# mitiko/weath3rb0i

Hardware: AMD Instinct MI355X
Metric: encode MiB/s, 64 KiB blocks, bit-exact vs CPU ref (higher is better)
Workload: dtype u32

## Files before the change

### weath3rb0i_amd/csrc/w3_predict.h

```cpp
#pragma once
#include "w3_device.h"
#include "../../include/w3hip.h"

namespace w3 {

#define W3_PF 8

#define W3_HALF_CU_LDS 81920u
template <int NW, size_t USED> struct HalfCuPad { static constexpr size_t words = (NW > 1 && USED < W3_HALF_CU_LDS) ? (W3_HALF_CU_LDS - USED + 3u) / 4u : (NW > 1 ? 0u : 1u); };
template <size_t WORDS> struct HalfCuPadDecl {
    static __device__ __forceinline__ void keep(uint64_t n) {
        __shared__ uint32_t pad_[WORDS];
        if (n == ~0ull) pad_[threadIdx.x % WORDS] = 1u;
    }
};
template <> struct HalfCuPadDecl<0> { static __device__ __forceinline__ void keep(uint64_t) {} };
#define W3_HALF_CU_PAD(NW, USED) HalfCuPadDecl<((NW) > 1 ? HalfCuPad<NW, (USED)>::words : 0u)>::keep(a.n);

struct PredictArgs {
    const uint8_t *in;
    uint64_t n;
    uint32_t block_size, nblocks;
    uint4 *P;
    const uint2 *keys;
    uint32_t *perm;
    uint2 *rec;
    uint4 *sink;
    const uint2 *rec_src;
    uint32_t *splits;
    uint32_t *job_counter;
    uint32_t hbits;
    uint32_t maxseg;
    uint32_t dbg_flags;
    unsigned long long *dbg;
    uint32_t fault_block;
};

#define W3_STAMP(slot)                                                                         \
    do {                                                                                       \
        if (a.dbg) {                                                                           \
            const unsigned long long t_ = __builtin_amdgcn_s_memtime();                        \
            if ((threadIdx.x & 63) == 0) atomicAdd(&a.dbg[slot], t_ - t_prev);                 \
            t_prev = t_;                                                                       \
        }                                                                                      \
    } while (0)

__device__ __forceinline__ uint64_t lane_lt_mask() { return (1ull << (threadIdx.x & 63)) - 1ull; }
__device__ __forceinline__ uint64_t lane_gt_mask() { return ~((2ull << (threadIdx.x & 63)) - 1ull); }

__device__ __forceinline__ uint32_t readlane_u32(uint32_t v, int k) { return (uint32_t)__builtin_amdgcn_readlane((int)v, k); }
__device__ __forceinline__ uint64_t readlane_u64(uint64_t v, int k) {
    uint32_t lo = readlane_u32((uint32_t)v, k), hi = readlane_u32((uint32_t)(v >> 32), k);
    return ((uint64_t)hi << 32) | lo;
}

template <int H>
__device__ __forceinline__ void match_windows(uint32_t w16, uint64_t M[8]) {
    uint64_t X[16];
#pragma unroll
    for (int b = 1; b < 16; b++) {
        if (b >= 1 && b <= 7 + H) {
            const bool mybit = (w16 >> b) & 1u;
            const uint64_t B = __ballot(mybit);
            X[b] = mybit ? B : ~B;
        }
    }
    if constexpr (H == 8) {
        uint64_t A2[15], A4[13];
#pragma unroll
        for (int b = 1; b <= 14; b++) A2[b] = X[b] & X[b + 1];
#pragma unroll
        for (int b = 1; b <= 12; b++) A4[b] = A2[b] & A2[b + 2];
#pragma unroll
        for (int j = 0; j < 8; j++) M[j] = A4[8 - j] & A4[12 - j];
    } else {
#pragma unroll
        for (int j = 0; j < 8; j++) {
            uint64_t m = ~0ull;
#pragma unroll
            for (int k = 0; k < H; k++) m &= X[8 - j + k];
            M[j] = m;
        }
    }
}

template <int H>
__device__ __forceinline__ void match_keys(uint2 k8, uint64_t M[8]) {
#pragma unroll
    for (int j = 0; j < 8; j++) {
        const uint32_t key = ((j < 4 ? k8.x : k8.y) >> (8 * (j & 3))) & 0xFFu;
        uint32_t mlo = 0xFFFFFFFFu, mhi = 0xFFFFFFFFu;
#pragma unroll
        for (int k = 0; k < H; k++) {
            const uint32_t sm = (uint32_t)__builtin_amdgcn_sbfe((int)key, k, 1);
            const uint64_t B = __ballot(sm != 0u);
            mlo &= ~((uint32_t)B ^ sm);
            mhi &= ~((uint32_t)(B >> 32) ^ sm);
        }
        M[j] = ((uint64_t)mhi << 32) | mlo;
    }
}

__device__ __forceinline__ uint32_t mbcnt64(uint64_t m) {
    return __builtin_amdgcn_mbcnt_hi((uint32_t)(m >> 32), __builtin_amdgcn_mbcnt_lo((uint32_t)m, 0u));
}

template <bool GROUPED>
__device__ __forceinline__ void rank_round(uint32_t c0, const uint32_t key[8], const uint64_t M[8], uint64_t seg, bool valid, bool rd,
                                           uint32_t *tbl, uint32_t p[8], uint32_t fin[8], uint32_t &wmask) {
    __asm__ volatile("" ::: "memory");
    const uint64_t gt = lane_gt_mask();
    const int lane = threadIdx.x & 63;
    wmask = 0u;
    uint32_t basev[8];
#pragma unroll
    for (int j = 0; j < 8; j++) basev[j] = tbl[j * 256 + key[j]];
#pragma unroll
    for (int j = 0; j < 8; j++) {
        const uint64_t Mj = M[j] & seg;
        const uint32_t bit = (c0 >> (7 - j)) & 1u;
        const uint64_t ones = __ballot(bit) & Mj;
        uint32_t base = basev[j];
        if constexpr (GROUPED) base = rd ? base : 0u;
        const uint32_t b0 = base & 0xFFFFu, b1 = base >> 16;
        const uint32_t n1l = mbcnt64(ones), n0l = mbcnt64(Mj) - n1l;
        uint32_t s0 = b0 + n0l, s1 = b1 + n1l;
        const bool last = valid && (Mj & gt) == 0ull;
        uint32_t f0 = s0 + (bit ^ 1u), f1 = s1 + bit;
        uint64_t satm = __ballot(last && (f0 >= 65535u || f1 >= 65535u));
        uint32_t f = f0 | (f1 << 16);
        while (satm) {
            const int k = __ffsll((long long)satm) - 1;
            const uint64_t Mc = readlane_u64(Mj, k);
            const uint64_t Oc = readlane_u64(ones, k);
            uint32_t st = readlane_u32(base, k);
            uint64_t it = Mc;
            while (it) {
                const int m = __ffsll((long long)it) - 1;
                it &= it - 1;
                if (lane == m) { s0 = st & 0xFFFFu; s1 = st >> 16; }
                st = counter_update_packed(st, (uint32_t)(Oc >> m) & 1u);
            }
            if (lane == k) f = st;
            satm &= satm - 1;
        }
        p[j] = counter_p(s0, s1);
        fin[j] = f;
        wmask |= last ? (1u << j) : 0u;
    }
    if constexpr (!GROUPED) {
#pragma unroll
        for (int j = 0; j < 8; j++)
            if ((wmask >> j) & 1u) tbl[j * 256 + key[j]] = fin[j];
        __asm__ volatile("" ::: "memory");
    }
}

#define W3_ATOMIC_LIM 65400u
#ifndef W3_ATOMIC_MAXSEG
#define W3_ATOMIC_MAXSEG 4u
#endif
typedef uint16_t w3_u16x2 __attribute__((ext_vector_type(2)));

__device__ __forceinline__ void atomic_round(uint32_t *tbl, uint32_t c0, const uint32_t key[8], bool on, uint32_t v[8]) {
#pragma unroll
    for (int j = 0; j < 8; j++) {
        const uint32_t inc = on ? (((c0 >> (7 - j)) & 1u) ? 0x10000u : 1u) : 0u;
        v[j] = __hip_atomic_fetch_add(&tbl[j * 256 + key[j]], inc, __ATOMIC_RELAXED, __HIP_MEMORY_SCOPE_WORKGROUP);
    }
}
__device__ __forceinline__ bool atomic_round_hot(const uint32_t v[8]) {
    w3_u16x2 m = __builtin_bit_cast(w3_u16x2, v[0]);
#pragma unroll
    for (int j = 1; j < 8; j++) m = __builtin_elementwise_max(m, __builtin_bit_cast(w3_u16x2, v[j]));
    return __ballot(max((uint32_t)m.x, (uint32_t)m.y) >= W3_ATOMIC_LIM) != 0ull;
}

__host__ __device__ __forceinline__ uint32_t lds_order_hash(uint32_t wave, uint32_t round, uint32_t lane) {
    uint32_t x = (wave * 64u + round) * 64u + lane + 0x9E3779B9u;
    x ^= x >> 16; x *= 0x7FEB352Du; x ^= x >> 15; x *= 0x846CA68Bu; x ^= x >> 16;
    return x;
}
__host__ __device__ __forceinline__ uint32_t lds_order_key(uint32_t wave, uint32_t h) {
    const uint32_t kind = wave & 3u;
    return kind == 0 ? 77u : kind == 1 ? (h & 7u) * 32u + 1u : kind == 2 ? (h & 255u) : (h & 2047u);
}
__global__ void __launch_bounds__(64) k_lds_order_selftest(uint32_t *old) {
    __shared__ uint32_t tbl[2048];
    const uint32_t lane = threadIdx.x;
    for (uint32_t i = lane; i < 2048u; i += 64u) tbl[i] = 0u;
    __builtin_amdgcn_wave_barrier();
    for (uint32_t r = 0; r < 32u; r++) {
        const uint32_t h = lds_order_hash(blockIdx.x, r, lane);
        old[(blockIdx.x * 32u + r) * 64u + lane] =
            __hip_atomic_fetch_add(&tbl[lds_order_key(blockIdx.x, h)], (h >> 20) & 1u ? 0x10000u : 1u, __ATOMIC_RELAXED, __HIP_MEMORY_SCOPE_WORKGROUP);
    }
}

__device__ __forceinline__ uint4 pack_p(const uint32_t p[8]) {
    return make_uint4(p[0] | (p[1] << 16), p[2] | (p[3] << 16), p[4] | (p[5] << 16), p[6] | (p[7] << 16));
}

__device__ __forceinline__ uint32_t mix_pair(uint32_t cur, uint32_t nw) {
    const uint32_t c_lo = cur & 0xFFFFu, c_hi = cur >> 16, n_lo = nw & 0xFFFFu, n_hi = nw >> 16;
    const uint32_t lo = opinion_dist(n_lo) > opinion_dist(c_lo) ? n_lo : c_lo;
    const uint32_t hi = opinion_dist(n_hi) > opinion_dist(c_hi) ? n_hi : c_hi;
    return lo | (hi << 16);
}
__device__ __forceinline__ uint4 mix_p(uint4 cur, uint4 nw) {
    return make_uint4(mix_pair(cur.x, nw.x), mix_pair(cur.y, nw.y), mix_pair(cur.z, nw.z), mix_pair(cur.w, nw.w));
}

#define W3_HD __host__ __device__ __forceinline__
#include "w3_verify.h"
#undef W3_HD
#include "w3_window.h"

template <int H, bool KEYS, int NW = 1>
__global__ void __launch_bounds__(64 * NW) k_predict_small(PredictArgs a) {
    __shared__ uint32_t tbl_[NW][8 * 256];
    __shared__ uint32_t st_w_[NW][W3_PF * 64];
    __shared__ uint2 st_k_[NW][KEYS ? W3_PF * 64 : 1];
    W3_HALF_CU_PAD(NW, sizeof(tbl_) + sizeof(st_w_) + sizeof(st_k_))
    const int lane = threadIdx.x & 63;
    const uint32_t wv = threadIdx.x >> 6;
    uint32_t *tbl = tbl_[wv], *st_w = st_w_[wv];
    uint2 *st_k = st_k_[wv];
    constexpr uint32_t KM = (1u << H) - 1u;
    for (uint32_t b = blockIdx.x * NW + wv; b < a.nblocks; b += gridDim.x * NW) {
        const uint64_t off = (uint64_t)b * a.block_size;
        const uint32_t len = (uint32_t)((a.n - off) < a.block_size ? (a.n - off) : a.block_size);
        const uint8_t *blk = a.in + off;
#pragma unroll
        for (int k = 0; k < 32; k++) tbl[k * 64 + lane] = 0u;
        __builtin_amdgcn_wave_barrier();
        bool exact = (a.dbg_flags & 2u) != 0u;
        const uint32_t first = window_head(off, 3u);
        const uint32_t last = len - 1u;
        uint32_t nw[W3_PF]; uint2 nk[W3_PF];
#pragma unroll
        for (int r = 0; r < W3_PF; r++) {
            const uint32_t ic = min((uint32_t)(r * 64 + lane), last);
            if constexpr (KEYS) { nk[r] = a.keys[off + ic]; nw[r] = blk[ic]; } else { nw[r] = load_window(blk, ic, first); nk[r] = make_uint2(0, 0); }
        }
        for (uint32_t bbase = 0; bbase < len; bbase += 64u * W3_PF) {
            __asm__ volatile("" ::: "memory");
            __builtin_amdgcn_wave_barrier();
#pragma unroll
            for (int r = 0; r < W3_PF; r++) { st_w[r * 64 + lane] = nw[r]; if constexpr (KEYS) st_k[r * 64 + lane] = nk[r]; }
            __asm__ volatile("" ::: "memory");
            __builtin_amdgcn_wave_barrier();
#pragma unroll
            for (int r = 0; r < W3_PF; r++) {
                const uint32_t ic = min(bbase + (uint32_t)((W3_PF + r) * 64 + lane), last);
                if constexpr (KEYS) { nk[r] = a.keys[off + ic]; nw[r] = blk[ic]; } else nw[r] = load_window(blk, ic, first);
            }
#pragma unroll 1
          for (uint32_t rr = 0; rr < W3_PF; rr++) {
            const uint32_t base = bbase + rr * 64u;
            if (base >= len) break;
            const uint32_t i = base + lane;
            const bool valid = i < len;
            const uint32_t w = st_w[rr * 64u + lane];
            uint2 k8 = make_uint2(0, 0);
            if constexpr (KEYS) k8 = st_k[rr * 64u + lane];
            uint32_t c0 = 0, key[8], p[8];
            if constexpr (KEYS) {
                c0 = valid ? w : 0u;
#pragma unroll
                for (int j = 0; j < 8; j++) key[j] = ((j < 4 ? k8.x : k8.y) >> (8 * (j & 3))) & KM;
            } else {
                const uint32_t wv = valid ? w : 0u;
                c0 = wv & 0xFFu;
#pragma unroll
                for (int j = 0; j < 8; j++) key[j] = ((wv & 0xFFFFu) >> (8 - j)) & KM;
            }
            if (!exact) {
                uint32_t v[8];
                __asm__ volatile("" ::: "memory");
                atomic_round(tbl, c0, key, valid, v);
                __asm__ volatile("" ::: "memory");
                if ((a.dbg_flags & 8u) && base == 64u && (a.fault_block == 0xFFFFFFFFu || a.fault_block == b)) v[0] = (uint32_t)__shfl_xor((int)v[0], 1, 64);
#pragma unroll
                for (int j = 0; j < 8; j++) p[j] = counter_p_packed(v[j]);
                exact = atomic_round_hot(v);
            } else {
                uint64_t M[8];
                if constexpr (KEYS) match_keys<H>(valid ? k8 : make_uint2(0, 0), M);
                else match_windows<H>((valid ? w : 0u) & 0xFFFFu, M);
                const uint64_t seg = __ballot(valid);
                uint32_t fin[8], wm;
                rank_round<false>(c0, key, M, seg, valid, true, tbl, p, fin, wm);
            }
            {
                uint4 *dst = valid ? a.P + (off + i) : a.sink + lane;
                *dst = pack_p(p);
            }
          }
        }
    }
}

__device__ __forceinline__ uint32_t wave_excl_scan_u32(uint32_t v, uint32_t *total) {
    const int lane = threadIdx.x & 63;
    uint32_t inc = v;
#pragma unroll
    for (int d = 1; d < 64; d <<= 1) {
        uint32_t o = __shfl_up(inc, d, 64);
        if (lane >= d) inc += o;
    }
    *total = __shfl(inc, 63, 64);
    return inc - v;
}


template <int NPASS, bool C2ONLY = false>
__device__ __forceinline__ void partition_hist(const uint8_t *blk, uint32_t len, uint32_t first, uint32_t *hist) {
    const int lane = threadIdx.x & 63;
    const uint64_t gt = lane_gt_mask();
    if (lane < 16 * NPASS) hist[lane] = 0u;
    __builtin_amdgcn_wave_barrier();
    uint32_t wn[W3_PF];
    const uint32_t last = len - 1u;
#pragma unroll
    for (int r = 0; r < W3_PF; r++) wn[r] = load_window(blk, min(r * 64u + lane, last), first);
    for (uint32_t base = 0; base < len; base += 64u * W3_PF) {
        uint32_t wc[W3_PF];
#pragma unroll
        for (int r = 0; r < W3_PF; r++) wc[r] = wn[r];
#pragma unroll
        for (int r = 0; r < W3_PF; r++) wn[r] = load_window(blk, min(base + (W3_PF + r) * 64u + lane, last), first);
#pragma unroll
        for (int r = 0; r < W3_PF; r++) {
            const uint32_t i = base + r * 64u + lane;
            if (base + r * 64u >= len) break;
            const bool valid = i < len;
            const uint32_t kb = valid ? (wc[r] >> 8) & 0xFFFFu : 0u;
            const uint64_t vm = __ballot(valid);
#pragma unroll
            for (int ps = 0; ps < NPASS; ps++) {
                const uint32_t d = C2ONLY ? (kb >> (8 + 4 * ps)) & 15u
                                 : NPASS == 4 ? ((ps < 2 ? (kb >> 8) : kb) >> (4 * (ps & 1))) & 15u : (kb >> (4 * ps)) & 15u;
                uint64_t m = vm;
#pragma unroll
                for (int k = 0; k < 4; k++) {
                    const bool mybit = (d >> k) & 1u;
                    const uint64_t B = __ballot(mybit);
                    m &= mybit ? B : ~B;
                }
                if (valid && (m & gt) == 0ull) hist[ps * 16 + d] += (uint32_t)__popcll(m);
                __asm__ volatile("" ::: "memory");
            }
        }
    }
    uint32_t v = lane < 16 * NPASS ? hist[lane] : 0u;
    uint32_t inc = v;
#pragma unroll
    for (int dd = 1; dd < 16; dd <<= 1) {
        uint32_t o = __shfl_up(inc, dd, 64);
        if ((lane & 15) >= dd) inc += o;
    }
    __builtin_amdgcn_wave_barrier();
    if (lane < 16 * NPASS) hist[lane] = inc - v;
    __builtin_amdgcn_wave_barrier();
}

template <bool FROM_INPUT>
__device__ __forceinline__ void partition_pass4(const uint8_t *blk, uint32_t len, uint32_t first, uint32_t back, uint32_t shift, const uint2 *src, uint2 *dst, uint32_t *bins) {
    const int lane = threadIdx.x & 63;
    const uint64_t gt = lane_gt_mask();
    const uint32_t last = len - 1u;
    uint2 rn[W3_PF];
#pragma unroll
    for (int r = 0; r < W3_PF; r++) {
        const uint32_t e = min(r * 64u + lane, last);
        if constexpr (FROM_INPUT) rn[r] = make_uint2(e, load_window(blk, e, first)); else rn[r] = src[e];
    }
    for (uint32_t base = 0; base < len; base += 64u * W3_PF) {
        uint2 rc[W3_PF];
#pragma unroll
        for (int r = 0; r < W3_PF; r++) rc[r] = rn[r];
#pragma unroll
        for (int r = 0; r < W3_PF; r++) {
            const uint32_t e = min(base + (W3_PF + r) * 64u + lane, last);
            if constexpr (FROM_INPUT) rn[r] = make_uint2(e, load_window(blk, e, first)); else rn[r] = src[e];
        }
#pragma unroll
        for (int r = 0; r < W3_PF; r++) {
            const uint32_t e = base + r * 64u + lane;
            if (base + r * 64u >= len) break;
            const bool valid = e < len;
            const uint2 rec = rc[r];
            const uint32_t d = valid ? (rec.y >> (8u * back + shift)) & 15u : 0u;
            uint64_t m = __ballot(valid);
#pragma unroll
            for (int k = 0; k < 4; k++) {
                const bool mybit = (d >> k) & 1u;
                const uint64_t B = __ballot(mybit);
                m &= mybit ? B : ~B;
            }
            if (valid) {
                const uint32_t bs = bins[d];
                dst[bs + mbcnt64(m)] = rec;
                if ((m & gt) == 0ull) bins[d] = bs + (uint32_t)__popcll(m);
            }
            __asm__ volatile("" ::: "memory");
        }
    }
}

#define W3_SLICES 64u

template <int NBYTES>
__global__ void __launch_bounds__(64) k_partition(PredictArgs a) {
    __shared__ uint32_t hist[64];
    const int lane = threadIdx.x;
    uint2 *perm_a = reinterpret_cast<uint2 *>(a.perm) + (uint64_t)blockIdx.x * 2u * a.block_size;
    uint2 *perm_b = perm_a + a.block_size;
    for (uint32_t b = blockIdx.x; b < a.nblocks; b += gridDim.x) {
        const uint64_t off = (uint64_t)b * a.block_size;
        const uint32_t len = (uint32_t)((a.n - off) < a.block_size ? (a.n - off) : a.block_size);
        const uint8_t *blk = a.in + off;
        uint2 *out = a.rec + off;
        unsigned long long t_prev = a.dbg ? __builtin_amdgcn_s_memtime() : 0ull;
        const uint32_t first = window_head(off, 3u);
        if constexpr (NBYTES == 3) partition_hist<2, true>(blk, len, first, hist); else partition_hist<2 * NBYTES>(blk, len, first, hist);
        W3_STAMP(0);
        if constexpr (NBYTES == 3) {
            partition_pass4<false>(blk, len, first, 2, 0, a.rec_src + off, perm_a, hist);
            __threadfence_block();
            W3_STAMP(1);
            partition_pass4<false>(blk, len, first, 2, 4, perm_a, out, hist + 16);
        } else if constexpr (NBYTES == 1) {
            partition_pass4<true>(blk, len, first, 1, 0, nullptr, perm_a, hist);
            __threadfence_block();
            W3_STAMP(1);
            partition_pass4<false>(blk, len, first, 1, 4, perm_a, out, hist + 16);
        } else {
            partition_pass4<true>(blk, len, first, 2, 0, nullptr, perm_a, hist);
            __threadfence_block();
            W3_STAMP(1);
            partition_pass4<false>(blk, len, first, 2, 4, perm_a, perm_b, hist + 16);
            __threadfence_block();
            partition_pass4<false>(blk, len, first, 1, 0, perm_b, perm_a, hist + 32);
            __threadfence_block();
            partition_pass4<false>(blk, len, first, 1, 4, perm_a, out, hist + 48);
        }
        __threadfence_block();
        W3_STAMP(2);
        uint32_t *sp = a.splits + (uint64_t)b * (W3_SLICES + 1u);
        uint32_t prev = 0u;
        if (lane == 0) { sp[0] = 0u; sp[W3_SLICES] = len; }
        for (uint32_t sl = 1; sl < W3_SLICES; sl++) {
            uint32_t start = max((uint32_t)((uint64_t)sl * len / W3_SLICES), prev), found = len;
            for (uint32_t base = start; base < len; base += 64) {
                const uint32_t e = base + lane;
                bool head = false;
                if (e < len) {
                    const uint32_t g = NBYTES == 1 ? ((out[e].y >> 8) & 0xFFu) : ((out[e].y >> 8) & 0xFFFFu);
                    const uint32_t gp = e ? (NBYTES == 1 ? ((out[e - 1].y >> 8) & 0xFFu) : ((out[e - 1].y >> 8) & 0xFFFFu)) : 0xFFFFFFFFu;
                    head = g != gp;
                }
                const uint64_t hm = __ballot(head);
                if (hm) { found = base + (uint32_t)(__ffsll((long long)hm) - 1); break; }
            }
            if (lane == 0) sp[sl] = found;
            prev = found;
        }
        W3_STAMP(4);
    }
}

#define W3_P8_TILE 2048u
#define W3_P8_ROUNDS (W3_P8_TILE / 64u)

__device__ __forceinline__ void wave_excl_scan_256(const uint32_t *cnt, uint32_t *excl, uint32_t *excl2, const uint32_t *base = nullptr, uint32_t *delta = nullptr) {
    const int lane = threadIdx.x & 63;
    const uint32_t c0 = cnt[4 * lane], c1 = cnt[4 * lane + 1], c2 = cnt[4 * lane + 2], c3 = cnt[4 * lane + 3];
    uint32_t g[4] = {0u, 0u, 0u, 0u};
    if (delta) for (int k = 0; k < 4; k++) g[k] = base[4 * lane + k];
    uint32_t tot;
    const uint32_t e0 = wave_excl_scan_u32(c0 + c1 + c2 + c3, &tot);
    const uint32_t e[4] = {e0, e0 + c0, e0 + c0 + c1, e0 + c0 + c1 + c2};
#pragma unroll
    for (int k = 0; k < 4; k++) {
        excl[4 * lane + k] = e[k];
        if (excl2) excl2[4 * lane + k] = e[k];
        if (delta) delta[4 * lane + k] = g[k] - e[k];
    }
}

template <int MODE, int NW = 1, bool FAULT = false>
__global__ void __launch_bounds__(64 * NW) k_partition8(PredictArgs a) {
    __shared__ uint2 tile_[NW][W3_P8_TILE];
    __shared__ uint32_t cnt_[NW][4][256];
    W3_HALF_CU_PAD(NW, sizeof(tile_) + sizeof(cnt_))
    const int lane = threadIdx.x & 63;
    const uint32_t wv = threadIdx.x >> 6;
    uint2 *tile = tile_[wv];
    uint32_t *gcur = cnt_[wv][0], *tcnt = cnt_[wv][1], *tstart = cnt_[wv][2], *gdelta = cnt_[wv][3], *tcur = cnt_[wv][3];
    constexpr uint32_t KSH = MODE == 1 ? 8u : 16u;
    for (uint32_t b = blockIdx.x * NW + wv; b < a.nblocks; b += gridDim.x * NW) {
        const uint64_t off = (uint64_t)b * a.block_size;
        const uint32_t len = (uint32_t)((a.n - off) < a.block_size ? (a.n - off) : a.block_size);
        const uint8_t *blk = a.in + off;
        const uint2 *src = MODE == 3 ? a.rec_src + off : nullptr;
        uint2 *out = a.rec + off;
        const uint32_t first = window_head(off, 3u);
        const uint32_t last = len - 1u;
        unsigned long long t_prev = a.dbg ? __builtin_amdgcn_s_memtime() : 0ull;
        constexpr uint32_t K = MODE == 1 ? 1u : 2u;
#pragma unroll
        for (int k = 0; k < 4; k++) tcnt[k * 64 + lane] = 0u;
        __builtin_amdgcn_wave_barrier();
        __asm__ volatile("" ::: "memory");
        {
            const uint32_t nbytes = len > K ? len - K : 0u;
            if (lane == 0) tcnt[0] = min(K, len);
            __builtin_amdgcn_wave_barrier();
            __asm__ volatile("" ::: "memory");
            if (len >= 16u) {
                const uint32_t cs_max = len - 16u;
                constexpr int HP = 4;
                uint4 qn[HP];
#pragma unroll
                for (int r = 0; r < HP; r++) __builtin_memcpy(&qn[r], blk + min((uint32_t)(r * 1024 + lane * 16), cs_max), 16);
                for (uint32_t base = 0; base < nbytes; base += 1024u * HP) {
                    uint4 qc[HP];
#pragma unroll
                    for (int r = 0; r < HP; r++) qc[r] = qn[r];
#pragma unroll
                    for (int r = 0; r < HP; r++) __builtin_memcpy(&qn[r], blk + min(base + (uint32_t)((HP + r) * 1024 + lane * 16), cs_max), 16);
#pragma unroll
                    for (int r = 0; r < HP; r++) {
                        const uint32_t want = base + (uint32_t)(r * 1024 + lane * 16), cs = min(want, cs_max);
                        const uint32_t w4[4] = {qc[r].x, qc[r].y, qc[r].z, qc[r].w};
#pragma unroll
                        for (int q = 0; q < 16; q++) {
                            const uint32_t pos = cs + (uint32_t)q;
                            if (pos >= want && pos < nbytes)
                                __hip_atomic_fetch_add(&tcnt[(w4[q >> 2] >> (8 * (q & 3))) & 0xFFu], 1u, __ATOMIC_RELAXED, __HIP_MEMORY_SCOPE_WORKGROUP);
                        }
                    }
                }
            } else {
                for (uint32_t pos = lane; pos < nbytes; pos += 64u)
                    __hip_atomic_fetch_add(&tcnt[blk[pos]], 1u, __ATOMIC_RELAXED, __HIP_MEMORY_SCOPE_WORKGROUP);
            }
        }
        __asm__ volatile("" ::: "memory");
        __builtin_amdgcn_wave_barrier();
        wave_excl_scan_256(tcnt, gcur, nullptr);
        __asm__ volatile("" ::: "memory");
        __builtin_amdgcn_wave_barrier();
        W3_STAMP(0);
        for (uint32_t t0 = 0; t0 < len; t0 += W3_P8_TILE) {
            const uint32_t tlen = min(W3_P8_TILE, len - t0);
            if (tlen == W3_P8_TILE) {
                uint32_t rx[MODE == 3 ? W3_P8_ROUNDS : 1u], ry[W3_P8_ROUNDS], rk[W3_P8_ROUNDS];
#pragma unroll
                for (uint32_t r = 0; r < W3_P8_ROUNDS; r++) {
                    const uint32_t e = t0 + r * 64u + lane;
                    if constexpr (MODE == 1) ry[r] = load_window(blk, e, first); else { const uint2 v = src[e]; rx[r] = v.x; ry[r] = v.y; }
                }
#pragma unroll
                for (int k = 0; k < 4; k++) tcnt[k * 64 + lane] = 0u;
                __asm__ volatile("" ::: "memory");
                __builtin_amdgcn_wave_barrier();
#pragma unroll
                for (uint32_t r = 0; r < W3_P8_ROUNDS; r++)
                    rk[r] = __hip_atomic_fetch_add(&tcnt[(ry[r] >> KSH) & 0xFFu], 1u, __ATOMIC_RELAXED, __HIP_MEMORY_SCOPE_WORKGROUP);
                if (FAULT && t0 == 0u && (a.fault_block == 0xFFFFFFFFu || a.fault_block == b)) {
                    const uint32_t d = (ry[1] >> KSH) & 0xFFu;
                    const uint32_t d_x = (uint32_t)__shfl_xor((int)d, 1, 64), rk_x = (uint32_t)__shfl_xor((int)rk[1], 1, 64);
                    if (d_x == d) rk[1] = rk_x;
                }
                __asm__ volatile("" ::: "memory");
                __builtin_amdgcn_wave_barrier();
                wave_excl_scan_256(tcnt, tstart, nullptr, gcur, gdelta);
                __asm__ volatile("" ::: "memory");
                __builtin_amdgcn_wave_barrier();
                W3_STAMP(1);
                uint32_t ts[W3_P8_ROUNDS];
#pragma unroll
                for (uint32_t r = 0; r < W3_P8_ROUNDS; r++) ts[r] = tstart[(ry[r] >> KSH) & 0xFFu];
                __asm__ volatile("" ::: "memory");
                __builtin_amdgcn_sched_barrier(0);
#pragma unroll
                for (uint32_t r = 0; r < W3_P8_ROUNDS; r++)
                    tile[ts[r] + rk[r]] = make_uint2(MODE == 1 ? t0 + r * 64u + lane : rx[r], ry[r]);
                __asm__ volatile("" ::: "memory");
                __builtin_amdgcn_wave_barrier();
                W3_STAMP(2);
                uint2 rc[W3_P8_ROUNDS];
#pragma unroll
                for (uint32_t r = 0; r < W3_P8_ROUNDS; r++) rc[r] = tile[r * 64u + lane];
                __asm__ volatile("" ::: "memory");
                __builtin_amdgcn_sched_barrier(0);
                uint32_t gd[W3_P8_ROUNDS];
#pragma unroll
                for (uint32_t r = 0; r < W3_P8_ROUNDS; r++) gd[r] = gdelta[(rc[r].y >> KSH) & 0xFFu];
                __asm__ volatile("" ::: "memory");
                __builtin_amdgcn_sched_barrier(0);
#pragma unroll
                for (uint32_t r = 0; r < W3_P8_ROUNDS; r++) out[gd[r] + (r * 64u + lane)] = rc[r];
            } else {
                uint2 rec[W3_P8_ROUNDS];
#pragma unroll
                for (uint32_t r = 0; r < W3_P8_ROUNDS; r++) {
                    const uint32_t e = min(t0 + r * 64u + lane, last);
                    if constexpr (MODE == 1) rec[r] = make_uint2(e, load_window(blk, e, first)); else rec[r] = src[e];
                }
#pragma unroll
                for (int k = 0; k < 4; k++) tcnt[k * 64 + lane] = 0u;
                __asm__ volatile("" ::: "memory");
                __builtin_amdgcn_wave_barrier();
#pragma unroll
                for (uint32_t r = 0; r < W3_P8_ROUNDS; r++)
                    if (r * 64u + lane < tlen) __hip_atomic_fetch_add(&tcnt[(rec[r].y >> KSH) & 0xFFu], 1u, __ATOMIC_RELAXED, __HIP_MEMORY_SCOPE_WORKGROUP);
                __asm__ volatile("" ::: "memory");
                __builtin_amdgcn_wave_barrier();
                wave_excl_scan_256(tcnt, tstart, tcur);
                __asm__ volatile("" ::: "memory");
                __builtin_amdgcn_wave_barrier();
                W3_STAMP(1);
#pragma unroll
                for (uint32_t r = 0; r < W3_P8_ROUNDS; r++) {
                    if (r * 64u + lane < tlen) {
                        uint32_t slot = __hip_atomic_fetch_add(&tcur[(rec[r].y >> KSH) & 0xFFu], 1u, __ATOMIC_RELAXED, __HIP_MEMORY_SCOPE_WORKGROUP);
                        if (FAULT && r == 1u && t0 == 0u && tlen >= 128u && (a.fault_block == 0xFFFFFFFFu || a.fault_block == b)) {
                            const uint32_t d = (rec[r].y >> KSH) & 0xFFu;
                            const uint32_t d_x = (uint32_t)__shfl_xor((int)d, 1, 64), slot_x = (uint32_t)__shfl_xor((int)slot, 1, 64);
                            if (d_x == d) slot = slot_x;
                        }
                        tile[slot] = rec[r];
                    }
                }
                __asm__ volatile("" ::: "memory");
                __builtin_amdgcn_wave_barrier();
                W3_STAMP(2);
#pragma unroll
                for (uint32_t r = 0; r < W3_P8_ROUNDS; r++) {
                    const uint32_t k = r * 64u + lane;
                    if (k < tlen) {
                        const uint2 rc = tile[k];
                        const uint32_t d = (rc.y >> KSH) & 0xFFu;
                        out[gcur[d] + (k - tstart[d])] = rc;
                    }
                }
            }
            __asm__ volatile("" ::: "memory");
            __builtin_amdgcn_wave_barrier();
#pragma unroll
            for (int k = 0; k < 4; k++) gcur[k * 64 + lane] += tcnt[k * 64 + lane];
            __asm__ volatile("" ::: "memory");
            __builtin_amdgcn_wave_barrier();
            W3_STAMP(5);
        }
        __threadfence_block();
        uint32_t *sp = a.splits + (uint64_t)b * (W3_SLICES + 1u);
        static_assert(W3_SLICES == 64u, "one lane per slice boundary");
        const uint32_t ideal = (uint32_t)((uint64_t)lane * len / W3_SLICES);
        uint32_t found;
        if constexpr (MODE == 1) {
            uint32_t lo = 0u, hi = 256u;
            while (lo < hi) {
                const uint32_t mid = (lo + hi) >> 1;
                const uint32_t st = mid == 0u ? 0u : gcur[mid - 1u];
                if (st >= ideal) hi = mid; else lo = mid + 1u;
            }
            found = lo == 0u ? 0u : gcur[lo - 1u];
        } else {
            found = 0xFFFFFFFFu;
            for (uint32_t s0 = 1; s0 < W3_SLICES; s0 += 8u) {
                uint32_t gy[8], gpy[8];
#pragma unroll
                for (int k = 0; k < 8; k++) {
                    const uint32_t st = readlane_u32(ideal, (int)min(s0 + (uint32_t)k, W3_SLICES - 1u));
                    const uint32_t e = min(st + lane, last);
                    gy[k] = out[e].y; gpy[k] = out[e ? e - 1u : 0u].y;
                }
#pragma unroll
                for (int k = 0; k < 8; k++) {
                    const uint32_t sl = s0 + (uint32_t)k;
                    if (sl >= W3_SLICES) break;
                    const uint32_t st = readlane_u32(ideal, (int)sl);
                    const uint32_t e = st + lane;
                    const bool head = e < len && (e == 0u || ((gy[k] >> 8) & 0xFFFFu) != ((gpy[k] >> 8) & 0xFFFFu));
                    const uint64_t hm = __ballot(head);
                    uint32_t f;
                    if (hm) f = st + (uint32_t)(__ffsll((long long)hm) - 1);
                    else {
                        const uint32_t before = readlane_u32(found, (int)sl - 1);
                        f = len;
                        if (sl > 1u && before != 0xFFFFFFFFu && before >= st) f = before;
                        else for (uint32_t base = st + 64u; base < len; base += 64u) {
                            const uint32_t e2 = base + lane;
                            const bool h2 = e2 < len && ((out[e2].y >> 8) & 0xFFFFu) != ((out[e2 - 1u].y >> 8) & 0xFFFFu);
                            const uint64_t hm2 = __ballot(h2);
                            if (hm2) { f = base + (uint32_t)(__ffsll((long long)hm2) - 1); break; }
                        }
                    }
                    if (lane == sl) found = f;
                }
            }
        }
        if (lane == 0) found = 0u;
        sp[lane] = found;
        if (lane == 0) sp[W3_SLICES] = len;
        W3_STAMP(4);
        if (a.dbg && lane == 0) atomicAdd(&a.dbg[6], 1ull);
    }
}

template <int NBYTES, int NW = 1, int PF = W3_PF, bool FAULT = false>
__global__ void __launch_bounds__(64 * NW) k_rank_sorted(PredictArgs a) {
    __shared__ uint32_t tbl_[NW][8 * 256];
    __shared__ uint2 st_r_[NW][PF * 64];
    W3_HALF_CU_PAD(NW, sizeof(tbl_) + sizeof(st_r_))
    const int lane = threadIdx.x & 63;
    uint32_t *tbl = tbl_[threadIdx.x >> 6];
    uint2 *st_r = st_r_[threadIdx.x >> 6];
    const uint32_t njobs = a.nblocks * W3_SLICES;
    for (;;) {
        uint32_t job = 0;
        if (lane == 0) job = atomicAdd(a.job_counter, 1u);
        job = __builtin_amdgcn_readfirstlane(job);
        if (job >= njobs) break;
        const uint32_t b = job / W3_SLICES, sl = job % W3_SLICES;
        const uint64_t off = (uint64_t)b * a.block_size;
        const uint32_t *sp = a.splits + (uint64_t)b * (W3_SLICES + 1u);
        const uint32_t lo = sp[sl], hi = sp[sl + 1];
        if (lo >= hi) continue;
        const uint32_t len = hi - lo;
        const uint2 *perm = a.rec + off + lo;
        unsigned long long t_prev = a.dbg ? __builtin_amdgcn_s_memtime() : 0ull;
#pragma unroll
        for (int k = 0; k < 32; k++) tbl[k * 64 + lane] = 0u;
        __builtin_amdgcn_wave_barrier();
        bool exact = (a.dbg_flags & 2u) != 0u;
        bool dirty = false;
        uint32_t open_g = 0xFFFFFFFFu;
        const uint32_t last = len - 1u;
        uint2 rn[PF];
#pragma unroll
        for (int r = 0; r < PF; r++) rn[r] = perm[min((uint32_t)(r * 64 + lane), last)];
        for (uint32_t bbase = 0; bbase < len; bbase += 64u * (uint32_t)PF) {
            __asm__ volatile("" ::: "memory");
            __builtin_amdgcn_wave_barrier();
#pragma unroll
            for (int r = 0; r < PF; r++) st_r[r * 64 + lane] = rn[r];
            __asm__ volatile("" ::: "memory");
            __builtin_amdgcn_wave_barrier();
#pragma unroll
            for (int r = 0; r < PF; r++) rn[r] = perm[min(bbase + (uint32_t)((PF + r) * 64 + lane), last)];
#pragma unroll 1
          for (uint32_t rr = 0; rr < (uint32_t)PF; rr++) {
            const uint32_t base = bbase + rr * 64u;
            if (base >= len) break;
            const uint32_t e = base + lane;
            const bool valid = e < len;
            const uint2 r_c = st_r[rr * 64u + lane];
            const uint32_t i = r_c.x; const uint32_t w = valid ? r_c.y : 0u;
            const uint32_t c0 = w & 0xFFu;
            const uint32_t g = NBYTES == 1 ? ((w >> 8) & 0xFFu) : ((w >> 8) & 0xFFFFu);
            const uint32_t ck = NBYTES == 1 ? ((w >> 16) & 0xFFu) : (w >> 24);
            const uint32_t w16 = (ck << 8) | c0;
            uint32_t gprev = __shfl_up(g, 1, 64);
            if (lane == 0) gprev = open_g;
            const uint64_t vm = __ballot(valid);
            const uint64_t heads = __ballot(valid && g != gprev) | 1ull;
            const uint64_t hle = heads & (lane_lt_mask() | (1ull << lane));
            const int start = 63 - __clzll((long long)hle);
            const uint64_t hgt = heads & lane_gt_mask();
            const uint64_t below_end = hgt ? ((1ull << (__ffsll((long long)hgt) - 1)) - 1ull) : ~0ull;
            const uint64_t seg = below_end & ~((1ull << start) - 1ull) & vm;
            uint32_t key[8], p[8];
#pragma unroll
            for (int j = 0; j < 8; j++) key[j] = (w16 >> (8 - j)) & 0xFFu;
            uint32_t *vt = tbl;
            const int lastlane = 63 - __clzll((long long)vm);
            const uint32_t g_last = readlane_u32(g, lastlane);
            uint64_t hm = heads & vm;
            if (!exact && (uint32_t)__popcll(hm) <= a.maxseg) {
                uint32_t v[8];
#pragma unroll
                for (int j = 0; j < 8; j++) v[j] = 0u;
                __asm__ volatile("" ::: "memory");
                if (dirty && readlane_u32(g, 0) != open_g) {
#pragma unroll
                    for (int k = 0; k < 32; k++) vt[k * 64 + lane] = 0u;
                    dirty = false;
                }
                bool carried = dirty;
                while (hm) {
                    const int st = __ffsll((long long)hm) - 1;
                    hm &= hm - 1ull;
                    const int en = hm ? __ffsll((long long)hm) - 1 : 64;
                    const bool in = valid && lane >= st && lane < en;
                    __asm__ volatile("" ::: "memory");
                    if (in) atomic_round(vt, c0, key, true, v);
                    __asm__ volatile("" ::: "memory");
                    if (hm) {
                        if (carried) {
#pragma unroll
                            for (int k = 0; k < 32; k++) vt[k * 64 + lane] = 0u;
                        } else if (in) {
#pragma unroll
                            for (int j = 0; j < 8; j++) vt[j * 256 + key[j]] = 0u;
                        }
                    }
                    carried = false;
                }
                __asm__ volatile("" ::: "memory");
                if constexpr (FAULT) {
                    if (64u - (lo + base) < 64u && (a.fault_block == 0xFFFFFFFFu || a.fault_block == b)) v[0] = (uint32_t)__shfl_xor((int)v[0], 1, 64);
                }
#pragma unroll
                for (int j = 0; j < 8; j++) p[j] = counter_p_packed(v[j]);
                exact = atomic_round_hot(v);
            } else {
                uint32_t fin[8], wm;
                uint64_t M[8];
                match_windows<8>(w16, M);
                rank_round<true>(c0, key, M, seg, valid, g == open_g, vt, p, fin, wm);
                if (g_last != open_g && dirty) {
#pragma unroll
                    for (int k = 0; k < 32; k++) vt[k * 64 + lane] = 0u;
                    dirty = false;
                }
                __builtin_amdgcn_wave_barrier();
                if (valid && g == g_last) {
#pragma unroll
                    for (int j = 0; j < 8; j++)
                        if ((wm >> j) & 1u) vt[j * 256 + key[j]] = fin[j];
                }
                __asm__ volatile("" ::: "memory");
                __builtin_amdgcn_wave_barrier();
            }
            dirty = true;
            open_g = g_last;
            {
                uint4 *dst = (valid && !(a.dbg_flags & 1u)) ? a.P + (off + ((a.dbg_flags & 4u) ? (i & 0xFFFu) : i)) : a.sink + lane;
                *dst = pack_p(p);
            }
          }
        }
        W3_STAMP(3);
        if (a.dbg && lane == 0 && sl == 0) atomicAdd(&a.dbg[7], 1ull);
    }
}

#define W3_HUFF_WALK 40u
struct HuffKeyArgs { const uint8_t *in; uint64_t n; uint32_t block_size; uint32_t hmask; const w3_huff_table *tb; uint2 *keys;
                     uint32_t *redo;
                     uint32_t nblocks;
                     uint32_t *keys32;  };

__device__ __forceinline__ void huff_hashes_of(uint32_t cb, uint32_t c0, const uint16_t *rcode, const uint8_t *rlen, uint32_t (&h)[8]) {
#pragma unroll
    for (int j = 0; j < 8; j++) {
        const uint32_t rem = (1u << j) | (c0 >> (8 - j));
        h[j] = (cb << rlen[rem]) | rcode[rem];
    }
}
template <bool WIDE>
__device__ __forceinline__ void huff_keys_store(const HuffKeyArgs &a, uint64_t g, uint32_t i, const uint32_t (&h)[8]) {
    if constexpr (WIDE) {
        uint4 *dst = reinterpret_cast<uint4 *>(a.keys32 + g * 8u);
        dst[0] = make_uint4(h[0], h[1], h[2], h[3]);
        dst[1] = make_uint4(h[4], h[5], h[6], h[7]);
    } else {
        uint32_t out[2] = {0u, 0u};
#pragma unroll
        for (int j = 0; j < 8; j++) {
            if (i == 0u && j == 0) continue;
            out[j >> 2] |= (h[j] & a.hmask & 0xFFu) << (8 * (j & 3));
        }
        a.keys[g] = make_uint2(out[0], out[1]);
    }
}

template <bool WIDE>
__global__ void __launch_bounds__(256) k_huffkeys(HuffKeyArgs a) {
    __shared__ uint16_t s_code[256], s_rcode[256];
    __shared__ uint8_t s_len[256], s_rlen[256];
    s_code[threadIdx.x] = a.tb->code[threadIdx.x]; s_len[threadIdx.x] = a.tb->len[threadIdx.x];
    s_rcode[threadIdx.x] = a.tb->rem_code[threadIdx.x]; s_rlen[threadIdx.x] = a.tb->rem_len[threadIdx.x];
    __syncthreads();
    const uint64_t g = (uint64_t)blockIdx.x * blockDim.x + threadIdx.x;
    if (g >= a.n) return;
    const uint64_t b = g / a.block_size;
    const uint32_t i = (uint32_t)(g - b * a.block_size);
    const uint8_t *blk = a.in + b * a.block_size;
    uint32_t cb = 0u, have = 0u, k = 1;
    for (; k <= i && have < 32u && k <= W3_HUFF_WALK; k++) {
        const uint32_t byte = blk[i - k];
        cb |= (uint32_t)s_code[byte] << have;
        have += s_len[byte];
    }
    if (have < 32u && k <= i) a.redo[b] = 1u;
    uint32_t h[8];
    huff_hashes_of(cb, blk[i], s_rcode, s_rlen, h);
    huff_keys_store<WIDE>(a, g, i, h);
}

template <bool WIDE>
__global__ void __launch_bounds__(64) k_huffkeys_fix(HuffKeyArgs a) {
    const uint32_t b = blockIdx.x * 64u + threadIdx.x;
    if (b >= a.nblocks || a.redo[b] == 0u) return;
    const uint64_t off = (uint64_t)b * a.block_size;
    const uint32_t len = (uint32_t)((a.n - off) < a.block_size ? (a.n - off) : a.block_size);
    uint32_t cb = 0u;
    for (uint32_t i = 0; i < len; i++) {
        const uint32_t c0 = a.in[off + i];
        uint32_t h[8];
        huff_hashes_of(cb, c0, a.tb->rem_code, a.tb->rem_len, h);
        huff_keys_store<WIDE>(a, off + i, i, h);
        const uint32_t l = a.tb->len[c0];
        cb = (l < 32u ? cb << l : 0u) | a.tb->code[c0];
    }
}

__global__ void __launch_bounds__(256) k_gather_blocks(const uint8_t *in, uint64_t n, uint32_t bs, uint32_t nb, uint32_t S, uint32_t rot, uint8_t *out) {
    const uint32_t s = blockIdx.y;
    const uint64_t src = (uint64_t)verify_block(rot, s, nb, S) * bs;
    const uint32_t len = (uint32_t)(n - src < bs ? n - src : bs);
    for (uint32_t i = blockIdx.x * 256u + threadIdx.x; i < len; i += gridDim.x * 256u) out[(uint64_t)s * bs + i] = in[src + i];
}
__global__ void __launch_bounds__(256) k_compare_blocks(const uint4 *main_p, const uint4 *ver_p, uint64_t n, uint32_t bs, uint32_t nb, uint32_t S, uint32_t rot, uint32_t *mismatch) {
    const uint32_t s = blockIdx.y;
    const uint64_t src = (uint64_t)verify_block(rot, s, nb, S) * bs;
    const uint32_t len = (uint32_t)(n - src < bs ? n - src : bs);
    uint32_t bad = 0;
    for (uint32_t i = blockIdx.x * 256u + threadIdx.x; i < len; i += gridDim.x * 256u) {
        const uint4 x = main_p[src + i], y = ver_p[(uint64_t)s * bs + i];
        bad |= (x.x ^ y.x) | (x.y ^ y.y) | (x.z ^ y.z) | (x.w ^ y.w);
    }
    if (__ballot(bad != 0u) && (threadIdx.x & 63u) == 0u) atomicAdd(mismatch, 1u);
}

struct MixArgs {
    const uint4 *src[16];
    int n_src;
    uint4 *P;
    uint64_t n;
};

__global__ void __launch_bounds__(256) k_mix(MixArgs a) {
    for (uint64_t g = (uint64_t)blockIdx.x * blockDim.x + threadIdx.x; g < a.n; g += (uint64_t)gridDim.x * blockDim.x) {
        uint4 acc = a.src[0][g];
        for (int l = 1; l < a.n_src; l++) acc = mix_p(acc, a.src[l][g]);
        a.P[g] = acc;
    }
}

struct HashArgs {
    const uint8_t *in; uint64_t n; uint32_t block_size; uint32_t max_bits; uint32_t hmask; uint16_t table[8]; uint2 *keys;
    uint4 *lut;
    uint16_t *lut_key;
};

__device__ __forceinline__ uint32_t sel8(const uint32_t (&v)[8], uint32_t k) {
    return k == 0 ? v[0] : k == 1 ? v[1] : k == 2 ? v[2] : k == 3 ? v[3] : k == 4 ? v[4] : k == 5 ? v[5] : k == 6 ? v[6] : v[7];
}

#define W3_ACHASH_LUT_BITS 16
__global__ void __launch_bounds__(256) k_achash_lut(HashArgs a) {
    const uint32_t e = blockIdx.x * blockDim.x + threadIdx.x;
    if (e >= (8u << W3_ACHASH_LUT_BITS)) return;
    const uint32_t v = e >> 3, j = e & 7u;
    uint32_t p32t[8], rot[8];
#pragma unroll
    for (int k = 0; k < 8; k++) p32t[k] = a.table[k] ? ((uint32_t)a.table[k] << 16) : 1u;
#pragma unroll
    for (int r = 0; r < 8; r++) {
        const uint32_t k = (j + 7u - (uint32_t)r) & 7u;
        rot[r] = k == 0 ? p32t[0] : k == 1 ? p32t[1] : k == 2 ? p32t[2] : k == 3 ? p32t[3] : k == 4 ? p32t[4] : k == 5 ? p32t[5] : k == 6 ? p32t[6] : p32t[7];
    }
    const ACHashState s = ac_history_hash_steps((uint64_t)v, a.max_bits, rot, ac_hash_state_init(a.max_bits), 0, W3_ACHASH_LUT_BITS);
    a.lut[e] = make_uint4(s.x1, s.x2, s.hash, s.meta);
    a.lut_key[e] = (uint16_t)((s.meta >> 31) ? (0x8000u | ((ac_hash_finish(s, a.max_bits) & a.hmask) & 0xFFu)) : 0u);
}

__global__ void __launch_bounds__(256) k_achash(HashArgs a) {
    __shared__ uint16_t q_id[4][512];
    __shared__ uint8_t q_key[4][64][8];
    const uint64_t g = (uint64_t)blockIdx.x * blockDim.x + threadIdx.x;
    const uint32_t wave = threadIdx.x >> 6, lane = threadIdx.x & 63u;
    const bool live = g < a.n;
    const uint64_t gc = live ? g : a.n - 1u;
    const uint64_t b = gc / a.block_size;
    const uint32_t i = (uint32_t)(gc - b * a.block_size);
    const uint8_t *blk = a.in + b * a.block_size;
    uint64_t hist0 = 0;
    for (uint32_t k = 1; k <= 8 && k <= i; k++) hist0 |= (uint64_t)blk[i - k] << (8 * (k - 1));
    const uint32_t c0 = blk[i];
    uint32_t p32t[8];
#pragma unroll
    for (int k = 0; k < 8; k++) p32t[k] = a.table[k] ? ((uint32_t)a.table[k] << 16) : 1u;
    uint32_t out[2] = {0, 0};
    uint32_t qn = 0, pend = 0;
    uint64_t hist = hist0;
#pragma unroll 1
    for (int j = 0; j < 8; j++) {
        const uint32_t t = i * 8u + j;
        bool pending = false;
        if (live && t != 0u) {
            const uint32_t le = a.lut_key[((uint32_t)hist & ((1u << W3_ACHASH_LUT_BITS) - 1u)) * 8u + (uint32_t)j];
            if (le & 0x8000u) out[j >> 2] |= (le & 0xFFu) << (8 * (j & 3));
            else pending = true;
        }
        const uint64_t pm = __ballot(pending);
        if (pending) { q_id[wave][qn + mbcnt64(pm)] = (uint16_t)((lane << 3) | (uint32_t)j); pend |= 1u << j; }
        qn += (uint32_t)__popcll(pm);
        hist = (hist << 1) | ((c0 >> (7 - j)) & 1u);
    }
    __asm__ volatile("" ::: "memory");
    __builtin_amdgcn_wave_barrier();
    for (uint32_t base = 0; base < qn; base += 64u) {
        const uint32_t e = base + lane;
        const uint32_t id = q_id[wave][min(e, qn - 1u)], j = id & 7u, owner = id >> 3;
        const uint32_t olo = (uint32_t)__shfl((int)(uint32_t)hist0, (int)owner, 64), ohi = (uint32_t)__shfl((int)(uint32_t)(hist0 >> 32), (int)owner, 64);
        const uint32_t oc0 = (uint32_t)__shfl((int)c0, (int)owner, 64);
        if (e < qn) {
            const uint64_t h = (((((uint64_t)ohi << 32) | olo)) << j) | (uint64_t)(oc0 >> (8u - j));
            const uint4 sv = a.lut[((uint32_t)h & ((1u << W3_ACHASH_LUT_BITS) - 1u)) * 8u + j];
            uint32_t rot[8];
#pragma unroll
            for (int r = 0; r < 8; r++) {
                const uint32_t k = (j + 7u - (uint32_t)r) & 7u;
                rot[r] = k == 0 ? p32t[0] : k == 1 ? p32t[1] : k == 2 ? p32t[2] : k == 3 ? p32t[3] : k == 4 ? p32t[4] : k == 5 ? p32t[5] : k == 6 ? p32t[6] : p32t[7];
            }
            ACHashState st; st.x1 = sv.x; st.x2 = sv.y; st.hash = sv.z; st.meta = sv.w;
            st = ac_history_hash_steps(h, a.max_bits, rot, st, W3_ACHASH_LUT_BITS, 64);
            q_key[wave][owner][j] = (uint8_t)(ac_hash_finish(st, a.max_bits) & a.hmask);
        }
    }
    __asm__ volatile("" ::: "memory");
    __builtin_amdgcn_wave_barrier();
#pragma unroll
    for (int j = 0; j < 8; j++)
        if ((pend >> j) & 1u) out[j >> 2] |= (uint32_t)q_key[wave][lane][j] << (8 * (j & 3));
    if (live) a.keys[g] = make_uint2(out[0], out[1]);
}

__global__ void __launch_bounds__(256) k_fill_half(uint4 *P, uint64_t n) {
    const uint64_t g = (uint64_t)blockIdx.x * blockDim.x + threadIdx.x;
    if (g < n) P[g] = make_uint4(0x80008000u, 0x80008000u, 0x80008000u, 0x80008000u);
}

}
```

Measured before the change: 14290.

## Software-pipeline rank round front-end one round ahead in k_rank_sorted

Moves the per-round decode (segment heads, keys, increments, group masks) into a RankFront struct computed one 64-record round ahead, and runs it inside the LDS atomic and rank_round latency windows through a callback with a sched_barrier. The prefetch offsets shift by two rounds to feed the lookahead. Atomic increments are precomputed per key and issued inline with workgroup-scope fetch_add. The goal is to hide the serial front-end ballots and shuffles behind LDS latency, at the cost of higher register pressure and more complex record staging.

```diff
diff --git a/profiles/rank_front_ahead/round_loop_rank_2_1_8.s b/profiles/rank_front_ahead/round_loop_rank_2_1_8.s
--- /dev/null
+++ b/profiles/rank_front_ahead/round_loop_rank_2_1_8.s
@@ -0,0 +1,1156 @@
+	s_lshl_b32 s41, s90, 6
+	s_or_b32 s40, s41, s89
+	s_cmp_lt_u32 s40, s57
+	s_waitcnt lgkmcnt(0)
+	v_mov_b64_e32 v[36:37], v[98:99]
+	s_mov_b32 s91, s93
+	v_mov_b32_e32 v70, v50
+	v_mov_b32_e32 v69, v68
+	v_mov_b64_e32 v[38:39], v[42:43]
+	s_cselect_b64 s[72:73], -1, 0
+	s_cmp_ge_u32 s40, s57
+	s_cbranch_scc1 .LBB161_41
+	v_cmp_lt_u32_e32 vcc, s56, v40
+	v_or_b32_e32 v2, s40, v0
+	s_or_b64 s[8:9], s[74:75], vcc
+	v_cmp_gt_u32_e64 s[6:7], s57, v2
+	s_and_b64 vcc, exec, s[8:9]
+	v_readfirstlane_b32 s12, v0
+	v_readfirstlane_b32 s13, v1
+	s_cbranch_vccnz .LBB161_42
+	s_andn2_b64 vcc, exec, s[78:79]
+	s_mov_b64 s[12:13], 0
+	s_cbranch_vccnz .LBB161_23
+	s_cmp_eq_u32 s94, s92
+	s_mov_b64 s[12:13], -1
+	s_cbranch_scc1 .LBB161_23
+	s_mov_b64 s[12:13], 0
+	ds_write2st64_b32 v53, v15, v15 offset1:1
+	ds_write2st64_b32 v53, v15, v15 offset0:2 offset1:3
+	ds_write2st64_b32 v53, v15, v15 offset0:4 offset1:5
+	ds_write2st64_b32 v53, v15, v15 offset0:6 offset1:7
+	ds_write2st64_b32 v53, v15, v15 offset0:8 offset1:9
+	ds_write2st64_b32 v53, v15, v15 offset0:10 offset1:11
+	ds_write2st64_b32 v53, v15, v15 offset0:12 offset1:13
+	ds_write2st64_b32 v53, v15, v15 offset0:14 offset1:15
+	ds_write2st64_b32 v53, v15, v15 offset0:16 offset1:17
+	ds_write2st64_b32 v53, v15, v15 offset0:18 offset1:19
+	ds_write2st64_b32 v53, v15, v15 offset0:20 offset1:21
+	ds_write2st64_b32 v53, v15, v15 offset0:22 offset1:23
+	ds_write2st64_b32 v53, v15, v15 offset0:24 offset1:25
+	ds_write2st64_b32 v53, v15, v15 offset0:26 offset1:27
+	ds_write2st64_b32 v53, v15, v15 offset0:28 offset1:29
+	ds_write2st64_b32 v53, v15, v15 offset0:30 offset1:31
+.LBB161_23:
+	s_and_b64 s[8:9], s[76:77], s[24:25]
+	s_cmp_eq_u64 s[8:9], 0
+	s_cbranch_scc1 .LBB161_43
+	s_add_u32 s10, s8, -1
+	s_addc_u32 s11, s9, -1
+	s_and_b64 s[10:11], s[10:11], s[8:9]
+	s_ff1_i32_b64 s14, s[8:9]
+	s_ff1_i32_b64 s8, s[10:11]
+	s_min_u32 s8, s8, 64
+	v_cmp_le_u32_e32 vcc, s14, v0
+	v_cmp_gt_u32_e64 s[8:9], s8, v0
+	s_and_b64 s[14:15], s[6:7], vcc
+	s_and_b64 s[8:9], s[14:15], s[8:9]
+	v_mov_b32_e32 v14, 0
+	v_mov_b32_e32 v40, 0
+	v_mov_b32_e32 v41, 0
+	v_mov_b32_e32 v52, 0
+	v_mov_b32_e32 v78, 0
+	v_mov_b32_e32 v79, 0
+	v_mov_b32_e32 v80, 0
+	v_mov_b32_e32 v81, 0
+	s_and_saveexec_b64 s[14:15], s[8:9]
+	s_cbranch_execz .LBB161_26
+	v_lshlrev_b32_e32 v2, 2, v54
+	ds_add_rtn_u32 v14, v2, v11
+	v_lshlrev_b32_e32 v2, 2, v77
+	ds_add_rtn_u32 v40, v2, v19 offset:1024
+	v_lshlrev_b32_e32 v2, 2, v76
+	ds_add_rtn_u32 v41, v2, v44 offset:2048
+	v_lshlrev_b32_e32 v2, 2, v75
+	ds_add_rtn_u32 v52, v2, v45 offset:3072
+	v_lshlrev_b32_e32 v2, 2, v74
+	ds_add_rtn_u32 v78, v2, v46 offset:4096
+	v_lshlrev_b32_e32 v2, 2, v73
+	ds_add_rtn_u32 v79, v2, v48 offset:5120
+	v_lshlrev_b32_e32 v2, 2, v72
+	ds_add_rtn_u32 v80, v2, v49 offset:6144
+	v_lshlrev_b32_e32 v2, 2, v51
+	ds_add_rtn_u32 v81, v2, v47 offset:7168
+.LBB161_26:
+	s_or_b64 exec, exec, s[14:15]
+	s_cmp_eq_u64 s[10:11], 0
+	s_cbranch_scc1 .LBB161_44
+	s_xor_b64 s[12:13], s[12:13], -1
+	s_andn2_b64 vcc, exec, s[12:13]
+	s_mov_b64 s[12:13], -1
+	s_cbranch_vccnz .LBB161_31
+	s_and_saveexec_b64 s[12:13], s[8:9]
+	s_cbranch_execz .LBB161_30
+	v_lshlrev_b32_e32 v2, 2, v54
+	ds_write_b32 v2, v15
+	v_lshlrev_b32_e32 v2, 2, v77
+	ds_write_b32 v2, v15 offset:1024
+	v_lshlrev_b32_e32 v2, 2, v76
+	ds_write_b32 v2, v15 offset:2048
+	v_lshlrev_b32_e32 v2, 2, v75
+	ds_write_b32 v2, v15 offset:3072
+	v_lshlrev_b32_e32 v2, 2, v74
+	ds_write_b32 v2, v15 offset:4096
+	v_lshlrev_b32_e32 v2, 2, v73
+	ds_write_b32 v2, v15 offset:5120
+	v_lshlrev_b32_e32 v2, 2, v72
+	ds_write_b32 v2, v15 offset:6144
+	v_lshlrev_b32_e32 v2, 2, v51
+	ds_write_b32 v2, v15 offset:7168
+.LBB161_30:
+	s_or_b64 exec, exec, s[12:13]
+	s_mov_b64 s[12:13], 0
+.LBB161_31:
+	s_andn2_b64 vcc, exec, s[12:13]
+	s_cbranch_vccnz .LBB161_33
+	ds_write2st64_b32 v53, v15, v15 offset1:1
+	ds_write2st64_b32 v53, v15, v15 offset0:2 offset1:3
+	ds_write2st64_b32 v53, v15, v15 offset0:4 offset1:5
+	ds_write2st64_b32 v53, v15, v15 offset0:6 offset1:7
+	ds_write2st64_b32 v53, v15, v15 offset0:8 offset1:9
+	ds_write2st64_b32 v53, v15, v15 offset0:10 offset1:11
+	ds_write2st64_b32 v53, v15, v15 offset0:12 offset1:13
+	ds_write2st64_b32 v53, v15, v15 offset0:14 offset1:15
+	ds_write2st64_b32 v53, v15, v15 offset0:16 offset1:17
+	ds_write2st64_b32 v53, v15, v15 offset0:18 offset1:19
+	ds_write2st64_b32 v53, v15, v15 offset0:20 offset1:21
+	ds_write2st64_b32 v53, v15, v15 offset0:22 offset1:23
+	ds_write2st64_b32 v53, v15, v15 offset0:24 offset1:25
+	ds_write2st64_b32 v53, v15, v15 offset0:26 offset1:27
+	ds_write2st64_b32 v53, v15, v15 offset0:28 offset1:29
+	ds_write2st64_b32 v53, v15, v15 offset0:30 offset1:31
+.LBB161_33:
+	v_lshlrev_b32_e32 v2, 2, v54
+	v_lshlrev_b32_e32 v3, 2, v77
+	v_lshlrev_b32_e32 v4, 2, v76
+	v_lshlrev_b32_e32 v5, 2, v75
+	v_lshlrev_b32_e32 v6, 2, v74
+	v_lshlrev_b32_e32 v7, 2, v73
+	v_lshlrev_b32_e32 v8, 2, v72
+	v_lshlrev_b32_e32 v9, 2, v51
+	s_branch .LBB161_35
+.LBB161_34:
+	s_or_b64 exec, exec, s[8:9]
+	s_cbranch_execz .LBB161_44
+	s_add_u32 s8, s10, -1
+	s_addc_u32 s9, s11, -1
+	s_ff1_i32_b64 s12, s[10:11]
+	s_and_b64 s[10:11], s[8:9], s[10:11]
+	s_ff1_i32_b64 s8, s[10:11]
+	s_min_u32 s8, s8, 64
+	v_cmp_le_u32_e32 vcc, s12, v0
+	v_cmp_gt_u32_e64 s[8:9], s8, v0
+	s_and_b64 s[12:13], s[6:7], vcc
+	s_and_b64 s[8:9], s[12:13], s[8:9]
+	s_and_saveexec_b64 s[12:13], s[8:9]
+	s_cbranch_execz .LBB161_37
+	s_waitcnt lgkmcnt(7)
+	ds_add_rtn_u32 v14, v2, v11
+	s_waitcnt lgkmcnt(7)
+	ds_add_rtn_u32 v40, v3, v19 offset:1024
+	s_waitcnt lgkmcnt(7)
+	ds_add_rtn_u32 v41, v4, v44 offset:2048
+	s_waitcnt lgkmcnt(7)
+	ds_add_rtn_u32 v52, v5, v45 offset:3072
+	s_waitcnt lgkmcnt(7)
+	ds_add_rtn_u32 v78, v6, v46 offset:4096
+	s_waitcnt lgkmcnt(7)
+	ds_add_rtn_u32 v79, v7, v48 offset:5120
+	s_waitcnt lgkmcnt(7)
+	ds_add_rtn_u32 v80, v8, v49 offset:6144
+	s_waitcnt lgkmcnt(7)
+	ds_add_rtn_u32 v81, v9, v47 offset:7168
+.LBB161_37:
+	s_or_b64 exec, exec, s[12:13]
+	s_cmp_eq_u64 s[10:11], 0
+	s_cbranch_scc1 .LBB161_40
+	s_and_saveexec_b64 s[12:13], s[8:9]
+	s_xor_b64 s[8:9], exec, s[12:13]
+	s_cbranch_execz .LBB161_34
+	ds_write_b32 v2, v15
+	ds_write_b32 v3, v15 offset:1024
+	ds_write_b32 v4, v15 offset:2048
+	ds_write_b32 v5, v15 offset:3072
+	ds_write_b32 v6, v15 offset:4096
+	ds_write_b32 v7, v15 offset:5120
+	ds_write_b32 v8, v15 offset:6144
+	ds_write_b32 v9, v15 offset:7168
+	s_branch .LBB161_34
+.LBB161_40:
+	s_branch .LBB161_44
+.LBB161_41:
+	s_mov_b64 s[8:9], s[74:75]
+	v_mov_b64_e32 v[98:99], v[36:37]
+	s_mov_b32 s93, s91
+	v_mov_b32_e32 v50, v70
+	v_mov_b32_e32 v68, v69
+	v_mov_b64_e32 v[42:43], v[38:39]
+	s_branch .LBB161_67
+.LBB161_42:
+	s_mov_b64 s[76:77], s[12:13]
+	s_mov_b64 s[24:25], s[12:13]
+	s_cbranch_execnz .LBB161_45
+	s_branch .LBB161_66
+.LBB161_43:
+	v_mov_b32_e32 v81, 0
+	v_mov_b32_e32 v80, 0
+	v_mov_b32_e32 v79, 0
+	v_mov_b32_e32 v78, 0
+	v_mov_b32_e32 v52, 0
+	v_mov_b32_e32 v41, 0
+	v_mov_b32_e32 v40, 0
+	v_mov_b32_e32 v14, 0
+.LBB161_44:
+	v_lshl_add_u32 v2, s41, 3, v65
+	s_add_i32 s8, s40, 64
+	ds_read_b64 v[98:99], v2
+	v_mov_b32_e32 v2, s8
+	v_sub_u32_e64 v2, s57, v2 clamp
+	v_cmp_lt_u32_e64 s[76:77], v0, v2
+	s_flbit_i32_b64 s22, s[76:77]
+	s_min_u32 s22, s22, 64
+	v_cndmask_b32_e64 v71, 0, v37, s[76:77]
+	v_lshrrev_b32_e32 v2, 8, v71
+	v_and_b32_e32 v68, 0xffff, v2
+	v_mov_b32_e32 v2, s91
+	s_not_b32 s22, s22
+	v_lshrrev_b32_e32 v11, 24, v71
+	v_mov_b32_dpp v2, v68 wave_shr:1 row_mask:0xf bank_mask:0xf
+	v_cmp_ne_u32_e32 vcc, v68, v2
+	s_and_b64 s[8:9], s[76:77], vcc
+	v_cndmask_b32_e64 v2, 0, 1, s[8:9]
+	v_cmp_ne_u32_e64 s[8:9], 0, v2
+	s_or_b32 s24, s8, 1
+	v_and_b32_e32 v3, s24, v10
+	v_and_b32_e32 v2, s9, v1
+	v_ffbh_u32_e32 v3, v3
+	v_add_u32_e64 v3, v3, 32 clamp
+	v_ffbh_u32_e32 v2, v2
+	v_min3_u32 v2, v3, v2, 64
+	v_and_b32_e32 v3, s9, v13
+	v_sub_u32_e32 v6, 63, v2
+	v_and_b32_e32 v2, s8, v12
+	v_ffbl_b32_e32 v4, v3
+	v_add_u32_e32 v4, 32, v4
+	v_ffbl_b32_e32 v5, v2
+	v_min_u32_e32 v4, v5, v4
+	v_lshlrev_b64 v[4:5], v4, -1
+	v_not_b32_e32 v4, v4
+	v_cmp_ne_u64_e32 vcc, 0, v[2:3]
+	v_lshlrev_b64 v[2:3], v6, -1
+	v_not_b32_e32 v5, v5
+	v_cndmask_b32_e32 v4, -1, v4, vcc
+	v_and_b32_e32 v42, v4, v2
+	v_and_b32_e32 v2, 0x80, v71
+	v_cndmask_b32_e32 v5, -1, v5, vcc
+	v_cmp_eq_u32_e32 vcc, 0, v2
+	v_and_b32_e32 v2, 64, v71
+	s_mov_b32 s25, s9
+	v_cmp_eq_u32_e64 s[8:9], 0, v2
+	v_and_b32_e32 v2, 32, v71
+	v_cmp_eq_u32_e64 s[10:11], 0, v2
+	v_and_b32_e32 v2, 16, v71
+	v_cmp_eq_u32_e64 s[12:13], 0, v2
+	v_and_b32_e32 v2, 8, v71
+	v_cmp_eq_u32_e64 s[14:15], 0, v2
+	v_and_b32_e32 v2, 4, v71
+	s_cmp_lg_u64 s[76:77], 0
+	v_cmp_eq_u32_e64 s[16:17], 0, v2
+	v_and_b32_e32 v2, 2, v71
+	s_cselect_b32 s22, s22, 0
+	v_and_b32_e32 v19, v5, v3
+	v_cmp_eq_u32_e64 s[18:19], 0, v2
+	v_and_b32_e32 v2, 1, v71
+	v_readlane_b32 s93, v68, s22
+	v_cmp_eq_u32_e64 s[20:21], 0, v2
+	s_and_b64 s[26:27], s[24:25], s[76:77]
+	s_waitcnt lgkmcnt(8)
+	v_and_b32_e32 v2, 0xffff, v14
+	v_lshrrev_b32_e32 v3, 16, v14
+	s_waitcnt lgkmcnt(7)
+	v_and_b32_e32 v4, 0xffff, v40
+	v_lshrrev_b32_e32 v5, 16, v40
+	v_add3_u32 v43, v2, v3, 2
+	v_add3_u32 v44, v4, v5, 2
+	v_cvt_f32_u32_e32 v2, v43
+	v_add_u32_e32 v45, 1, v3
+	v_cvt_f32_u32_e32 v3, v44
+	v_add_u32_e32 v46, 1, v5
+	v_rcp_iflag_f32_e32 v2, v2
+	v_cvt_f32_u32_e32 v5, v46
+	v_cvt_f32_u32_e32 v4, v45
+	v_rcp_iflag_f32_e32 v3, v3
+	s_mov_b32 s22, 0x3ef0a3d7
+	s_waitcnt lgkmcnt(6)
+	v_lshrrev_b32_e32 v7, 16, v41
+	s_waitcnt lgkmcnt(5)
+	v_and_b32_e32 v6, 0xffff, v52
+	v_pk_mul_f32 v[2:3], v[2:3], v[4:5]
+	v_mov_b64_e32 v[4:5], s[22:23]
+	v_pk_fma_f32 v[2:3], v[2:3], s[50:51], v[4:5] op_sel_hi:[1,0,0]
+	v_lshrrev_b32_e32 v8, 16, v52
+	v_cvt_u32_f32_e32 v47, v3
+	v_and_b32_e32 v3, 0xffff, v41
+	v_add3_u32 v48, v3, v7, 2
+	v_cvt_f32_u32_e32 v3, v48
+	v_add3_u32 v49, v6, v8, 2
+	v_add_u32_e32 v50, 1, v7
+	v_add_u32_e32 v82, 1, v8
+	v_rcp_iflag_f32_e32 v6, v3
+	v_cvt_f32_u32_e32 v3, v49
+	v_cvt_f32_u32_e32 v9, v82
+	v_cvt_f32_u32_e32 v8, v50
+	v_cvt_u32_f32_e32 v83, v2
+	v_rcp_iflag_f32_e32 v7, v3
+	v_lshlrev_b32_e32 v84, 1, v44
+	v_lshlrev_b32_e32 v92, 1, v49
+	v_lshlrev_b32_e32 v85, 1, v43
+	v_pk_mul_f32 v[2:3], v[6:7], v[8:9]
+	s_waitcnt lgkmcnt(4)
+	v_lshrrev_b32_e32 v7, 16, v78
+	v_pk_fma_f32 v[2:3], v[2:3], s[50:51], v[4:5] op_sel_hi:[1,0,0]
+	s_waitcnt lgkmcnt(3)
+	v_and_b32_e32 v6, 0xffff, v79
+	v_cvt_u32_f32_e32 v86, v3
+	v_and_b32_e32 v3, 0xffff, v78
+	v_add3_u32 v87, v3, v7, 2
+	v_cvt_f32_u32_e32 v3, v87
+	v_lshrrev_b32_e32 v8, 16, v79
+	v_add3_u32 v88, v6, v8, 2
+	v_add_u32_e32 v89, 1, v7
+	v_rcp_iflag_f32_e32 v6, v3
+	v_cvt_f32_u32_e32 v3, v88
+	v_add_u32_e32 v90, 1, v8
+	v_cvt_f32_u32_e32 v9, v90
+	v_cvt_f32_u32_e32 v8, v89
+	v_rcp_iflag_f32_e32 v7, v3
+	v_cvt_u32_f32_e32 v91, v2
+	v_lshlrev_b32_e32 v93, 1, v48
+	v_lshlrev_b32_e32 v102, 1, v88
+	v_pk_mul_f32 v[2:3], v[6:7], v[8:9]
+	s_waitcnt lgkmcnt(2)
+	v_lshrrev_b32_e32 v7, 16, v80
+	v_pk_fma_f32 v[2:3], v[2:3], s[50:51], v[4:5] op_sel_hi:[1,0,0]
+	s_waitcnt lgkmcnt(1)
+	v_and_b32_e32 v6, 0xffff, v81
+	v_cvt_u32_f32_e32 v94, v3
+	v_and_b32_e32 v3, 0xffff, v80
+	v_add3_u32 v95, v3, v7, 2
+	v_cvt_f32_u32_e32 v3, v95
+	v_lshrrev_b32_e32 v8, 16, v81
+	v_add3_u32 v96, v6, v8, 2
+	v_add_u32_e32 v97, 1, v7
+	v_rcp_iflag_f32_e32 v6, v3
+	v_cvt_f32_u32_e32 v3, v96
+	v_add_u32_e32 v100, 1, v8
+	v_cvt_f32_u32_e32 v9, v100
+	v_cvt_f32_u32_e32 v8, v97
+	v_rcp_iflag_f32_e32 v7, v3
+	v_cvt_u32_f32_e32 v101, v2
+	v_lshlrev_b32_e32 v103, 1, v87
+	v_pk_max_u16 v14, v14, v40
+	v_pk_mul_f32 v[2:3], v[6:7], v[8:9]
+	v_lshl_add_u32 v7, v46, 17, v44
+	v_pk_fma_f32 v[2:3], v[2:3], s[50:51], v[4:5] op_sel_hi:[1,0,0]
+	v_lshlrev_b32_e32 v4, 1, v96
+	v_cvt_u32_f32_e32 v3, v3
+	v_cvt_u32_f32_e32 v2, v2
+	v_lshl_add_u32 v44, v90, 17, v88
+	v_lshl_add_u32 v46, v100, 17, v96
+	v_mul_u32_u24_e32 v90, v3, v4
+	v_lshlrev_b32_e32 v5, 1, v95
+	v_sub_u32_e32 v46, v46, v90
+	v_lshl_add_u32 v6, v45, 17, v43
+	v_lshl_add_u32 v9, v82, 17, v49
+	v_lshl_add_u32 v43, v89, 17, v87
+	v_lshl_add_u32 v45, v97, 17, v95
+	v_mul_u32_u24_e32 v82, v86, v92
+	v_mul_u32_u24_e32 v89, v2, v5
+	v_cmp_ge_u32_e64 s[22:23], v46, v4
+	v_sub_u32_e32 v45, v45, v89
+	v_sub_u32_e32 v82, v9, v82
+	v_addc_co_u32_e64 v9, s[22:23], 0, v3, s[22:23]
+	v_lshl_add_u32 v8, v50, 17, v48
+	v_mul_u32_u24_e32 v50, v91, v93
+	v_mul_u32_u24_e32 v88, v94, v102
+	v_cmp_ge_u32_e64 s[22:23], v45, v5
+	v_sub_u32_e32 v44, v44, v88
+	v_sub_u32_e32 v50, v8, v50
+	v_addc_co_u32_e64 v8, s[22:23], 0, v2, s[22:23]
+	v_mul_u32_u24_e32 v49, v47, v84
+	v_mul_u32_u24_e32 v87, v101, v103
+	v_cmp_ge_u32_e64 s[22:23], v44, v102
+	v_sub_u32_e32 v43, v43, v87
+	v_sub_u32_e32 v49, v7, v49
+	v_addc_co_u32_e64 v7, s[22:23], 0, v94, s[22:23]
+	v_mul_u32_u24_e32 v48, v83, v85
+	v_cmp_ge_u32_e64 s[22:23], v43, v103
+	v_pk_max_u16 v14, v14, v41
+	v_sub_u32_e32 v48, v6, v48
+	v_addc_co_u32_e64 v6, s[22:23], 0, v101, s[22:23]
+	v_pk_max_u16 v14, v14, v52
+	v_cmp_ge_u32_e64 s[22:23], v82, v92
+	v_pk_max_u16 v14, v14, v78
+	v_and_b32_e32 v43, s77, v19
+	v_addc_co_u32_e64 v5, s[22:23], 0, v86, s[22:23]
+	v_pk_max_u16 v14, v14, v79
+	v_cmp_ge_u32_e64 s[22:23], v50, v93
+	v_pk_max_u16 v14, v14, v80
+	v_and_b32_e32 v50, 0xff, v71
+	v_addc_co_u32_e64 v4, s[22:23], 0, v91, s[22:23]
+	v_pk_max_u16 v14, v14, v81
+	v_cmp_ge_u32_e64 s[22:23], v49, v84
+	v_cndmask_b32_e64 v19, v67, 1, s[8:9]
+	v_max_u16_sdwa v14, v14, v14 dst_sel:DWORD dst_unused:UNUSED_PAD src0_sel:DWORD src1_sel:WORD_1
+	s_movk_i32 s8, 0xff77
+	v_addc_co_u32_e64 v3, s[22:23], 0, v47, s[22:23]
+	v_lshl_or_b32 v82, v11, 8, v50
+	v_cndmask_b32_e64 v11, v67, 1, vcc
+	s_bcnt1_i32_b64 s58, s[26:27]
+	v_cmp_lt_u16_e32 vcc, s8, v14
+	v_cmp_ge_u32_e64 s[22:23], v48, v85
+	s_cmp_lg_u64 vcc, 0
+	v_and_b32_e32 v42, s76, v42
+	v_addc_co_u32_e64 v2, s[22:23], 0, v83, s[22:23]
+	v_cndmask_b32_e64 v44, v67, 1, s[10:11]
+	v_cndmask_b32_e64 v45, v67, 1, s[12:13]
+	v_cndmask_b32_e64 v46, v67, 1, s[14:15]
+	v_cndmask_b32_e64 v48, v67, 1, s[16:17]
+	v_cndmask_b32_e64 v49, v67, 1, s[18:19]
+	v_cndmask_b32_e64 v47, v67, 1, s[20:21]
+	v_readlane_b32 s94, v68, 0
+	s_cselect_b64 s[8:9], -1, 0
+	v_mov_b64_e32 v[40:41], s[58:59]
+	s_branch .LBB161_66
+.LBB161_45:
+	v_and_b32_e32 v4, 2, v70
+	v_cmp_ne_u32_e64 s[10:11], 0, v4
+	v_and_b32_e32 v4, 4, v70
+	v_cmp_ne_u32_e64 s[16:17], 0, v4
+	v_and_b32_e32 v4, 8, v70
+	v_cmp_ne_u32_e64 s[20:21], 0, v4
+	v_and_b32_e32 v4, 16, v70
+	v_cmp_ne_u32_e64 s[24:25], 0, v4
+	v_and_b32_e32 v4, 32, v70
+	v_cmp_ne_u32_e64 s[28:29], 0, v4
+	v_and_b32_e32 v4, 64, v70
+	v_cmp_ne_u32_e64 s[34:35], 0, v4
+	v_and_b32_e32 v4, 0x80, v70
+	v_lshlrev_b32_e32 v2, 8, v54
+	v_cmp_ne_u32_e64 s[38:39], 0, v4
+	v_bfe_u32 v4, v70, 7, 1
+	s_movk_i32 s12, 0x100
+	v_cmp_ne_u32_e64 s[36:37], 0, v4
+	v_bitop3_b32 v4, v70, s12, v2 bitop3:0xc8
+	v_cmp_eq_u32_e64 s[12:13], 0, v4
+	v_or_b32_e32 v3, v70, v2
+	v_bfe_u32 v5, v3, 8, 1
+	v_cndmask_b32_e64 v4, 0, -1, s[12:13]
+	s_movk_i32 s12, 0x200
+	v_bitop3_b32 v6, v70, s12, v2 bitop3:0xc8
+	v_cmp_ne_u32_e32 vcc, 0, v5
+	v_bfe_u32 v7, v3, 9, 1
+	v_cmp_eq_u32_e64 s[12:13], 0, v6
+	v_xor_b32_e32 v5, vcc_hi, v4
+	v_xor_b32_e32 v4, vcc_lo, v4
+	v_cmp_ne_u32_e32 vcc, 0, v7
+	v_cndmask_b32_e64 v6, 0, -1, s[12:13]
+	s_movk_i32 s12, 0x400
+	v_xor_b32_e32 v19, vcc_hi, v6
+	v_xor_b32_e32 v40, vcc_lo, v6
+	v_bitop3_b32 v6, v70, s12, v2 bitop3:0xc8
+	v_bfe_u32 v7, v3, 10, 1
+	v_cmp_eq_u32_e64 s[12:13], 0, v6
+	v_cmp_ne_u32_e32 vcc, 0, v7
+	v_bfe_u32 v7, v3, 11, 1
+	v_cndmask_b32_e64 v6, 0, -1, s[12:13]
+	s_movk_i32 s12, 0x800
+	v_xor_b32_e32 v41, vcc_hi, v6
+	v_xor_b32_e32 v44, vcc_lo, v6
+	v_bitop3_b32 v6, v70, s12, v2 bitop3:0xc8
+	v_cmp_eq_u32_e64 s[12:13], 0, v6
+	v_cmp_ne_u32_e32 vcc, 0, v7
+	v_bfe_u32 v7, v3, 12, 1
+	v_cndmask_b32_e64 v6, 0, -1, s[12:13]
+	s_movk_i32 s12, 0x1000
+	v_xor_b32_e32 v43, vcc_hi, v6
+	v_xor_b32_e32 v46, vcc_lo, v6
+	v_bitop3_b32 v6, v70, s12, v2 bitop3:0xc8
+	v_cmp_eq_u32_e64 s[12:13], 0, v6
+	v_cmp_ne_u32_e32 vcc, 0, v7
+	v_bfe_u32 v7, v3, 13, 1
+	v_cndmask_b32_e64 v6, 0, -1, s[12:13]
+	s_movk_i32 s12, 0x2000
+	v_xor_b32_e32 v45, vcc_hi, v6
+	v_xor_b32_e32 v48, vcc_lo, v6
+	v_bitop3_b32 v6, v70, s12, v2 bitop3:0xc8
+	v_cmp_eq_u32_e64 s[12:13], 0, v6
+	v_lshlrev_b32_e32 v81, 2, v54
+	v_lshlrev_b32_e32 v78, 2, v77
+	v_lshlrev_b32_e32 v77, 2, v76
+	v_lshlrev_b32_e32 v76, 2, v75
+	v_lshlrev_b32_e32 v75, 2, v74
+	v_lshlrev_b32_e32 v74, 2, v73
+	v_lshlrev_b32_e32 v73, 2, v72
+	v_lshlrev_b32_e32 v72, 2, v51
+	v_lshl_add_u32 v51, s41, 3, v65
+	s_add_i32 s40, s40, 64
+	v_cmp_ne_u32_e32 vcc, 0, v7
+	v_cndmask_b32_e64 v6, 0, -1, s[12:13]
+	s_movk_i32 s12, 0x4000
+	ds_read_b32 v80, v81
+	ds_read_b32 v95, v78 offset:1024
+	ds_read_b32 v94, v77 offset:2048
+	ds_read_b32 v93, v76 offset:3072
+	ds_read_b32 v92, v75 offset:4096
+	ds_read_b32 v89, v74 offset:5120
+	ds_read_b32 v86, v73 offset:6144
+	ds_read_b32 v83, v72 offset:7168
+	s_waitcnt lgkmcnt(8)
+	ds_read_b64 v[98:99], v51
+	v_mov_b32_e32 v51, s40
+	v_xor_b32_e32 v47, vcc_hi, v6
+	v_xor_b32_e32 v50, vcc_lo, v6
+	v_bitop3_b32 v6, v70, s12, v2 bitop3:0xc8
+	v_sub_u32_e64 v51, s57, v51 clamp
+	v_cmp_eq_u32_e64 s[12:13], 0, v6
+	v_cmp_lt_u32_e64 s[76:77], v0, v51
+	v_bfe_u32 v7, v3, 14, 1
+	v_cndmask_b32_e64 v6, 0, -1, s[12:13]
+	s_mov_b32 s12, 0x8000
+	v_cndmask_b32_e64 v71, 0, v37, s[76:77]
+	v_bitop3_b32 v2, v70, s12, v2 bitop3:0xc8
+	v_lshrrev_b32_e32 v37, 8, v71
+	v_cmp_ne_u32_e32 vcc, 0, v7
+	v_bfe_u32 v3, v3, 15, 1
+	v_cmp_eq_u32_e64 s[12:13], 0, v2
+	v_and_b32_e32 v68, 0xffff, v37
+	v_mov_b32_e32 v37, s91
+	v_xor_b32_e32 v49, vcc_hi, v6
+	v_xor_b32_e32 v52, vcc_lo, v6
+	v_cmp_ne_u32_e32 vcc, 0, v3
+	v_cndmask_b32_e64 v2, 0, -1, s[12:13]
+	v_mov_b32_dpp v37, v68 wave_shr:1 row_mask:0xf bank_mask:0xf
+	v_xor_b32_e32 v42, vcc_hi, v2
+	v_xor_b32_e32 v79, vcc_lo, v2
+	v_cmp_ne_u32_e32 vcc, v68, v37
+	s_and_b64 s[40:41], s[76:77], vcc
+	v_cndmask_b32_e64 v37, 0, 1, s[40:41]
+	s_flbit_i32_b64 s40, s[76:77]
+	s_min_u32 s40, s40, 64
+	s_not_b32 s40, s40
+	s_cmp_lg_u64 s[76:77], 0
+	v_bfe_u32 v84, v70, 1, 1
+	v_bfe_u32 v87, v70, 2, 1
+	v_bfe_u32 v90, v70, 3, 1
+	v_bfe_u32 v91, v70, 4, 1
+	v_bfe_u32 v88, v70, 5, 1
+	v_bfe_u32 v85, v70, 6, 1
+	v_and_b32_e32 v7, v19, v5
+	v_and_b32_e32 v6, v40, v4
+	v_and_b32_e32 v9, v43, v41
+	v_and_b32_e32 v8, v46, v44
+	s_cselect_b32 s40, s40, 0
+	v_cmp_ne_u32_e64 s[8:9], 0, v84
+	v_cmp_ne_u32_e64 s[14:15], 0, v87
+	v_cmp_ne_u32_e64 s[18:19], 0, v90
+	v_cmp_ne_u32_e64 s[22:23], 0, v91
+	v_cmp_ne_u32_e64 s[26:27], 0, v88
+	v_cmp_ne_u32_e64 s[30:31], 0, v85
+	v_and_b32_e32 v11, v47, v45
+	v_and_b32_e32 v14, v50, v48
+	v_and_b32_e32 v3, v9, v7
+	v_and_b32_e32 v2, v8, v6
+	v_cmp_eq_u32_e64 s[12:13], s92, v69
+	v_cmp_ne_u32_e64 s[80:81], 0, v37
+	v_readlane_b32 s93, v68, s40
+	v_readlane_b32 s94, v68, 0
+	v_and_b32_e32 v37, v39, v42
+	v_and_b32_e32 v42, v38, v79
+	v_and_b32_e32 v42, v42, v2
+	v_and_b32_e32 v37, v37, v3
+	v_and_b32_e32 v42, v42, v52
+	s_movk_i32 s40, 0x7f
+	v_and_b32_e32 v37, v37, v49
+	v_and_b32_e32 v54, v42, v14
+	v_cmp_lt_u32_e32 vcc, s40, v70
+	v_and_b32_e32 v51, v37, v11
+	s_waitcnt lgkmcnt(8)
+	v_cndmask_b32_e64 v96, 0, v80, s[12:13]
+	v_and_b32_e32 v42, vcc_lo, v54
+	v_and_b32_e32 v37, vcc_hi, v51
+	v_mbcnt_lo_u32_b32 v79, v42, 0
+	v_mbcnt_lo_u32_b32 v80, v54, 0
+	v_mbcnt_hi_u32_b32 v79, v37, v79
+	v_mbcnt_hi_u32_b32 v80, v51, v80
+	v_sub_u32_e32 v80, v80, v79
+	v_lshrrev_b32_e32 v82, 7, v70
+	v_add_u32_sdwa v80, v80, v96 dst_sel:DWORD dst_unused:UNUSED_PAD src0_sel:DWORD src1_sel:WORD_0
+	v_add_u32_sdwa v79, v79, v96 dst_sel:DWORD dst_unused:UNUSED_PAD src0_sel:DWORD src1_sel:WORD_1
+	v_and_b32_e32 v101, v51, v13
+	v_and_b32_e32 v100, v54, v12
+	v_xad_u32 v97, v82, 1, v80
+	v_add_u32_e32 v82, v79, v82
+	v_cmp_eq_u64_e32 vcc, 0, v[100:101]
+	v_max_u32_e32 v100, v97, v82
+	s_and_b64 s[82:83], s[6:7], vcc
+	v_cmp_lt_u32_e32 vcc, s45, v100
+	s_and_b64 s[40:41], s[82:83], vcc
+	v_cndmask_b32_e64 v100, 0, 1, s[40:41]
+	v_cmp_ne_u32_e32 vcc, 0, v100
+	v_lshl_or_b32 v82, v82, 16, v97
+	s_cbranch_vccnz .LBB161_70
+.LBB161_46:
+	v_cndmask_b32_e64 v96, 0, 1, s[38:39]
+	v_mov_b32_e32 v97, s59
+	v_lshl_add_u64 v[96:97], v[96:97], 0, -1
+	v_xor_b32_e32 v54, s36, v96
+	v_xor_b32_e32 v51, s37, v97
+	v_and_b32_e32 v42, v4, v54
+	v_and_b32_e32 v40, v44, v40
+	v_and_b32_e32 v37, v5, v51
+	v_and_b32_e32 v19, v41, v19
+	v_and_b32_e32 v4, v40, v42
+	v_and_b32_e32 v41, v45, v43
+	v_and_b32_e32 v5, v19, v37
+	v_and_b32_e32 v45, v4, v38
+	v_and_b32_e32 v44, v48, v46
+	v_and_b32_e32 v43, v5, v39
+	v_and_b32_e32 v45, v45, v50
+	v_and_b32_e32 v43, v43, v47
+	v_and_b32_e32 v45, v45, v44
+	v_and_b32_e32 v43, v43, v41
+	v_and_b32_e32 v46, v45, v52
+	v_cmp_ne_u32_e32 vcc, 0, v85
+	v_and_b32_e32 v43, v43, v49
+	v_mbcnt_lo_u32_b32 v50, v46, 0
+	v_and_b32_e32 v48, vcc_lo, v46
+	v_and_b32_e32 v45, vcc_hi, v43
+	v_mbcnt_lo_u32_b32 v49, v48, 0
+	v_mbcnt_hi_u32_b32 v49, v45, v49
+	v_mbcnt_hi_u32_b32 v50, v43, v50
+	s_waitcnt lgkmcnt(7)
+	v_cndmask_b32_e64 v47, 0, v95, s[12:13]
+	v_sub_u32_e32 v50, v50, v49
+	v_add_u32_sdwa v52, v50, v47 dst_sel:DWORD dst_unused:UNUSED_PAD src0_sel:DWORD src1_sel:WORD_0
+	v_add_u32_sdwa v49, v49, v47 dst_sel:DWORD dst_unused:UNUSED_PAD src0_sel:DWORD src1_sel:WORD_1
+	v_and_b32_e32 v97, v43, v13
+	v_and_b32_e32 v96, v46, v12
+	v_xad_u32 v50, v85, 1, v52
+	v_add_u32_e32 v85, v49, v85
+	v_cmp_eq_u64_e32 vcc, 0, v[96:97]
+	v_max_u32_e32 v95, v50, v85
+	s_and_b64 s[38:39], s[6:7], vcc
+	v_cmp_lt_u32_e32 vcc, s45, v95
+	s_and_b64 s[36:37], s[38:39], vcc
+	v_cndmask_b32_e64 v95, 0, 1, s[36:37]
+	v_cmp_ne_u32_e32 vcc, 0, v95
+	v_lshl_or_b32 v85, v85, 16, v50
+	s_cbranch_vccnz .LBB161_73
+.LBB161_47:
+	v_cndmask_b32_e64 v46, 0, 1, s[34:35]
+	v_mov_b32_e32 v47, s59
+	v_lshl_add_u64 v[46:47], v[46:47], 0, -1
+	v_xor_b32_e32 v48, s30, v46
+	v_xor_b32_e32 v45, s31, v47
+	v_and_b32_e32 v46, v54, v48
+	v_and_b32_e32 v43, v51, v45
+	v_and_b32_e32 v6, v6, v46
+	v_and_b32_e32 v7, v7, v43
+	v_and_b32_e32 v50, v6, v38
+	v_and_b32_e32 v47, v7, v39
+	v_and_b32_e32 v8, v50, v8
+	v_and_b32_e32 v9, v47, v9
+	v_and_b32_e32 v8, v8, v14
+	v_cmp_ne_u32_e32 vcc, 0, v88
+	v_and_b32_e32 v9, v9, v11
+	v_mbcnt_lo_u32_b32 v51, v8, 0
+	v_and_b32_e32 v14, vcc_lo, v8
+	v_and_b32_e32 v11, vcc_hi, v9
+	v_mbcnt_lo_u32_b32 v50, v14, 0
+	v_mbcnt_hi_u32_b32 v50, v11, v50
+	v_mbcnt_hi_u32_b32 v51, v9, v51
+	s_waitcnt lgkmcnt(6)
+	v_cndmask_b32_e64 v47, 0, v94, s[12:13]
+	v_sub_u32_e32 v51, v51, v50
+	v_add_u32_sdwa v54, v51, v47 dst_sel:DWORD dst_unused:UNUSED_PAD src0_sel:DWORD src1_sel:WORD_0
+	v_add_u32_sdwa v51, v50, v47 dst_sel:DWORD dst_unused:UNUSED_PAD src0_sel:DWORD src1_sel:WORD_1
+	v_and_b32_e32 v95, v9, v13
+	v_and_b32_e32 v94, v8, v12
+	v_xad_u32 v50, v88, 1, v54
+	v_add_u32_e32 v88, v51, v88
+	v_cmp_eq_u64_e32 vcc, 0, v[94:95]
+	v_max_u32_e32 v94, v50, v88
+	s_and_b64 s[34:35], s[6:7], vcc
+	v_cmp_lt_u32_e32 vcc, s45, v94
+	s_and_b64 s[30:31], s[34:35], vcc
+	v_cndmask_b32_e64 v94, 0, 1, s[30:31]
+	v_cmp_ne_u32_e32 vcc, 0, v94
+	v_lshl_or_b32 v88, v88, 16, v50
+	s_cbranch_vccnz .LBB161_76
+.LBB161_48:
+	v_cndmask_b32_e64 v8, 0, 1, s[28:29]
+	v_mov_b32_e32 v9, s59
+	v_lshl_add_u64 v[8:9], v[8:9], 0, -1
+	v_xor_b32_e32 v47, s27, v9
+	v_xor_b32_e32 v50, s26, v8
+	v_and_b32_e32 v11, v45, v47
+	v_and_b32_e32 v14, v48, v50
+	v_and_b32_e32 v9, v37, v11
+	v_and_b32_e32 v8, v42, v14
+	v_and_b32_e32 v37, v9, v39
+	v_and_b32_e32 v42, v8, v38
+	v_and_b32_e32 v19, v37, v19
+	v_and_b32_e32 v37, v42, v40
+	v_and_b32_e32 v40, v37, v44
+	v_cmp_ne_u32_e32 vcc, 0, v91
+	v_and_b32_e32 v19, v19, v41
+	v_mbcnt_lo_u32_b32 v45, v40, 0
+	v_and_b32_e32 v42, vcc_lo, v40
+	v_and_b32_e32 v37, vcc_hi, v19
+	v_mbcnt_lo_u32_b32 v44, v42, 0
+	v_mbcnt_hi_u32_b32 v44, v37, v44
+	v_mbcnt_hi_u32_b32 v45, v19, v45
+	s_waitcnt lgkmcnt(5)
+	v_cndmask_b32_e64 v41, 0, v93, s[12:13]
+	v_sub_u32_e32 v45, v45, v44
+	v_add_u32_sdwa v48, v45, v41 dst_sel:DWORD dst_unused:UNUSED_PAD src0_sel:DWORD src1_sel:WORD_0
+	v_add_u32_sdwa v45, v44, v41 dst_sel:DWORD dst_unused:UNUSED_PAD src0_sel:DWORD src1_sel:WORD_1
+	v_and_b32_e32 v95, v19, v13
+	v_and_b32_e32 v94, v40, v12
+	v_xad_u32 v44, v91, 1, v48
+	v_add_u32_e32 v91, v45, v91
+	v_cmp_eq_u64_e32 vcc, 0, v[94:95]
+	v_max_u32_e32 v93, v44, v91
+	s_and_b64 s[28:29], s[6:7], vcc
+	v_cmp_lt_u32_e32 vcc, s45, v93
+	s_and_b64 s[26:27], s[28:29], vcc
+	v_cndmask_b32_e64 v93, 0, 1, s[26:27]
+	v_cmp_ne_u32_e32 vcc, 0, v93
+	v_lshl_or_b32 v91, v91, 16, v44
+	s_cbranch_vccnz .LBB161_79
+.LBB161_49:
+	v_cndmask_b32_e64 v40, 0, 1, s[24:25]
+	v_mov_b32_e32 v41, s59
+	v_lshl_add_u64 v[40:41], v[40:41], 0, -1
+	v_xor_b32_e32 v44, s22, v40
+	v_xor_b32_e32 v41, s23, v41
+	v_and_b32_e32 v40, v50, v44
+	v_and_b32_e32 v19, v47, v41
+	v_and_b32_e32 v42, v40, v38
+	v_and_b32_e32 v37, v19, v39
+	v_and_b32_e32 v42, v42, v46
+	v_and_b32_e32 v37, v37, v43
+	v_and_b32_e32 v2, v42, v2
+	v_cmp_ne_u32_e32 vcc, 0, v90
+	v_and_b32_e32 v3, v37, v3
+	v_mbcnt_lo_u32_b32 v46, v2, 0
+	v_and_b32_e32 v42, vcc_lo, v2
+	v_and_b32_e32 v37, vcc_hi, v3
+	v_mbcnt_lo_u32_b32 v43, v42, 0
+	v_mbcnt_hi_u32_b32 v43, v37, v43
+	v_mbcnt_hi_u32_b32 v46, v3, v46
+	s_waitcnt lgkmcnt(4)
+	v_cndmask_b32_e64 v50, 0, v92, s[12:13]
+	v_sub_u32_e32 v46, v46, v43
+	v_add_u32_sdwa v46, v46, v50 dst_sel:DWORD dst_unused:UNUSED_PAD src0_sel:DWORD src1_sel:WORD_0
+	v_add_u32_sdwa v43, v43, v50 dst_sel:DWORD dst_unused:UNUSED_PAD src0_sel:DWORD src1_sel:WORD_1
+	v_and_b32_e32 v93, v3, v13
+	v_and_b32_e32 v92, v2, v12
+	v_xad_u32 v47, v90, 1, v46
+	v_add_u32_e32 v90, v43, v90
+	v_cmp_eq_u64_e32 vcc, 0, v[92:93]
+	v_max_u32_e32 v92, v47, v90
+	s_and_b64 s[24:25], s[6:7], vcc
+	v_cmp_lt_u32_e32 vcc, s45, v92
+	s_and_b64 s[22:23], s[24:25], vcc
+	v_cndmask_b32_e64 v92, 0, 1, s[22:23]
+	v_cmp_ne_u32_e32 vcc, 0, v92
+	v_lshl_or_b32 v47, v90, 16, v47
+	s_cbranch_vccnz .LBB161_82
+.LBB161_50:
+	v_cndmask_b32_e64 v2, 0, 1, s[20:21]
+	v_mov_b32_e32 v3, s59
+	v_lshl_add_u64 v[2:3], v[2:3], 0, -1
+	v_xor_b32_e32 v42, s18, v2
+	v_xor_b32_e32 v37, s19, v3
+	v_and_b32_e32 v2, v44, v42
+	v_and_b32_e32 v3, v41, v37
+	v_and_b32_e32 v44, v2, v38
+	v_and_b32_e32 v41, v3, v39
+	v_and_b32_e32 v14, v44, v14
+	v_and_b32_e32 v11, v41, v11
+	v_and_b32_e32 v4, v14, v4
+	v_cmp_ne_u32_e32 vcc, 0, v87
+	v_and_b32_e32 v5, v11, v5
+	v_mbcnt_lo_u32_b32 v44, v4, 0
+	v_and_b32_e32 v14, vcc_lo, v4
+	v_and_b32_e32 v11, vcc_hi, v5
+	v_mbcnt_lo_u32_b32 v41, v14, 0
+	v_mbcnt_hi_u32_b32 v41, v11, v41
+	v_mbcnt_hi_u32_b32 v44, v5, v44
+	s_waitcnt lgkmcnt(3)
+	v_cndmask_b32_e64 v89, 0, v89, s[12:13]
+	v_sub_u32_e32 v44, v44, v41
+	v_add_u32_sdwa v44, v44, v89 dst_sel:DWORD dst_unused:UNUSED_PAD src0_sel:DWORD src1_sel:WORD_0
+	v_add_u32_sdwa v41, v41, v89 dst_sel:DWORD dst_unused:UNUSED_PAD src0_sel:DWORD src1_sel:WORD_1
+	v_and_b32_e32 v93, v5, v13
+	v_and_b32_e32 v92, v4, v12
+	v_xad_u32 v50, v87, 1, v44
+	v_add_u32_e32 v87, v41, v87
+	v_cmp_eq_u64_e32 vcc, 0, v[92:93]
+	v_max_u32_e32 v90, v50, v87
+	s_and_b64 s[20:21], s[6:7], vcc
+	v_cmp_lt_u32_e32 vcc, s45, v90
+	s_and_b64 s[18:19], s[20:21], vcc
+	v_cndmask_b32_e64 v90, 0, 1, s[18:19]
+	v_cmp_ne_u32_e32 vcc, 0, v90
+	v_lshl_or_b32 v50, v87, 16, v50
+	s_cbranch_vccnz .LBB161_85
+.LBB161_51:
+	v_cndmask_b32_e64 v4, 0, 1, s[16:17]
+	v_mov_b32_e32 v5, s59
+	v_lshl_add_u64 v[4:5], v[4:5], 0, -1
+	v_xor_b32_e32 v4, s14, v4
+	v_xor_b32_e32 v5, s15, v5
+	v_and_b32_e32 v14, v4, v38
+	v_and_b32_e32 v11, v5, v39
+	v_and_b32_e32 v14, v14, v42
+	v_and_b32_e32 v11, v11, v37
+	v_and_b32_e32 v14, v14, v40
+	v_and_b32_e32 v11, v11, v19
+	v_and_b32_e32 v6, v14, v6
+	v_cmp_ne_u32_e32 vcc, 0, v84
+	v_and_b32_e32 v7, v11, v7
+	v_mbcnt_lo_u32_b32 v37, v6, 0
+	v_and_b32_e32 v14, vcc_lo, v6
+	v_and_b32_e32 v11, vcc_hi, v7
+	v_mbcnt_lo_u32_b32 v19, v14, 0
+	v_mbcnt_hi_u32_b32 v19, v11, v19
+	v_mbcnt_hi_u32_b32 v37, v7, v37
+	s_waitcnt lgkmcnt(2)
+	v_cndmask_b32_e64 v42, 0, v86, s[12:13]
+	v_sub_u32_e32 v37, v37, v19
+	v_add_u32_sdwa v37, v37, v42 dst_sel:DWORD dst_unused:UNUSED_PAD src0_sel:DWORD src1_sel:WORD_0
+	v_add_u32_sdwa v19, v19, v42 dst_sel:DWORD dst_unused:UNUSED_PAD src0_sel:DWORD src1_sel:WORD_1
+	v_and_b32_e32 v87, v7, v13
+	v_and_b32_e32 v86, v6, v12
+	v_xad_u32 v40, v84, 1, v37
+	v_add_u32_e32 v84, v19, v84
+	v_cmp_eq_u64_e32 vcc, 0, v[86:87]
+	v_max_u32_e32 v86, v40, v84
+	s_and_b64 s[16:17], s[6:7], vcc
+	v_cmp_lt_u32_e32 vcc, s45, v86
+	s_and_b64 s[14:15], s[16:17], vcc
+	v_cndmask_b32_e64 v86, 0, 1, s[14:15]
+	v_cmp_ne_u32_e32 vcc, 0, v86
+	v_lshl_or_b32 v40, v84, 16, v40
+	s_cbranch_vccnz .LBB161_88
+.LBB161_52:
+	v_cndmask_b32_e64 v6, 0, 1, s[10:11]
+	v_mov_b32_e32 v7, s59
+	v_lshl_add_u64 v[6:7], v[6:7], 0, -1
+	v_xor_b32_e32 v6, s8, v6
+	v_xor_b32_e32 v7, s9, v7
+	v_and_b32_e32 v6, v38, v6
+	v_and_b32_e32 v7, v39, v7
+	v_and_b32_e32 v4, v6, v4
+	v_and_b32_e32 v5, v7, v5
+	v_and_b32_e32 v2, v4, v2
+	v_and_b32_e32 v6, 1, v70
+	v_and_b32_e32 v3, v5, v3
+	v_and_b32_e32 v2, v2, v8
+	v_cmp_ne_u32_e32 vcc, 0, v6
+	v_and_b32_e32 v3, v3, v9
+	v_mbcnt_lo_u32_b32 v9, v2, 0
+	v_and_b32_e32 v4, vcc_lo, v2
+	v_and_b32_e32 v5, vcc_hi, v3
+	v_mbcnt_lo_u32_b32 v8, v4, 0
+	v_mbcnt_hi_u32_b32 v8, v5, v8
+	v_mbcnt_hi_u32_b32 v9, v3, v9
+	s_waitcnt lgkmcnt(1)
+	v_cndmask_b32_e64 v7, 0, v83, s[12:13]
+	v_sub_u32_e32 v9, v9, v8
+	v_add_u32_sdwa v9, v9, v7 dst_sel:DWORD dst_unused:UNUSED_PAD src0_sel:DWORD src1_sel:WORD_0
+	v_add_u32_sdwa v8, v8, v7 dst_sel:DWORD dst_unused:UNUSED_PAD src0_sel:DWORD src1_sel:WORD_1
+	v_and_b32_e32 v39, v3, v13
+	v_and_b32_e32 v38, v2, v12
+	v_xad_u32 v11, v6, 1, v9
+	v_add_u32_e32 v6, v8, v6
+	v_cmp_eq_u64_e32 vcc, 0, v[38:39]
+	v_max_u32_e32 v14, v11, v6
+	s_and_b64 s[10:11], s[6:7], vcc
+	v_cmp_lt_u32_e32 vcc, s45, v14
+	s_and_b64 s[8:9], s[10:11], vcc
+	v_cndmask_b32_e64 v14, 0, 1, s[8:9]
+	v_cmp_ne_u32_e32 vcc, 0, v14
+	v_lshl_or_b32 v6, v6, 16, v11
+	s_cbranch_vccnz .LBB161_91
+.LBB161_53:
+	s_cmp_lg_u32 s91, s92
+	s_cselect_b64 s[8:9], -1, 0
+	s_and_b64 s[8:9], s[8:9], s[78:79]
+	s_andn2_b64 vcc, exec, s[8:9]
+	s_cbranch_vccnz .LBB161_55
+	ds_write2st64_b32 v53, v15, v15 offset1:1
+	ds_write2st64_b32 v53, v15, v15 offset0:2 offset1:3
+	ds_write2st64_b32 v53, v15, v15 offset0:4 offset1:5
+	ds_write2st64_b32 v53, v15, v15 offset0:6 offset1:7
+	ds_write2st64_b32 v53, v15, v15 offset0:8 offset1:9
+	ds_write2st64_b32 v53, v15, v15 offset0:10 offset1:11
+	ds_write2st64_b32 v53, v15, v15 offset0:12 offset1:13
+	ds_write2st64_b32 v53, v15, v15 offset0:14 offset1:15
+	ds_write2st64_b32 v53, v15, v15 offset0:16 offset1:17
+	ds_write2st64_b32 v53, v15, v15 offset0:18 offset1:19
+	ds_write2st64_b32 v53, v15, v15 offset0:20 offset1:21
+	ds_write2st64_b32 v53, v15, v15 offset0:22 offset1:23
+	ds_write2st64_b32 v53, v15, v15 offset0:24 offset1:25
+	ds_write2st64_b32 v53, v15, v15 offset0:26 offset1:27
+	ds_write2st64_b32 v53, v15, v15 offset0:28 offset1:29
+	ds_write2st64_b32 v53, v15, v15 offset0:30 offset1:31
+.LBB161_55:
+	v_cmp_eq_u32_e32 vcc, s91, v69
+	s_and_b64 s[12:13], s[6:7], vcc
+	s_and_saveexec_b64 s[8:9], s[12:13]
+	s_cbranch_execz .LBB161_65
+	s_and_saveexec_b64 s[12:13], s[82:83]
+	s_cbranch_execnz .LBB161_93
+	s_or_b64 exec, exec, s[12:13]
+	s_and_saveexec_b64 s[12:13], s[38:39]
+	s_cbranch_execnz .LBB161_94
+.LBB161_58:
+	s_or_b64 exec, exec, s[12:13]
+	s_and_saveexec_b64 s[12:13], s[34:35]
+	s_cbranch_execnz .LBB161_95
+.LBB161_59:
+	s_or_b64 exec, exec, s[12:13]
+	s_and_saveexec_b64 s[12:13], s[28:29]
+	s_cbranch_execnz .LBB161_96
+.LBB161_60:
+	s_or_b64 exec, exec, s[12:13]
+	s_and_saveexec_b64 s[12:13], s[24:25]
+	s_cbranch_execnz .LBB161_97
+.LBB161_61:
+	s_or_b64 exec, exec, s[12:13]
+	s_and_saveexec_b64 s[12:13], s[20:21]
+	s_cbranch_execnz .LBB161_98
+.LBB161_62:
+	s_or_b64 exec, exec, s[12:13]
+	s_and_saveexec_b64 s[12:13], s[16:17]
+	s_cbranch_execnz .LBB161_99
+.LBB161_63:
+	s_or_b64 exec, exec, s[12:13]
+	s_and_b64 exec, exec, s[10:11]
+.LBB161_64:
+	ds_write_b32 v72, v6 offset:7168
+.LBB161_65:
+	s_or_b64 exec, exec, s[8:9]
+	v_add3_u32 v2, v79, v80, 2
+	v_cvt_f32_u32_e32 v3, v2
+	v_add_u32_e32 v4, 1, v79
+	v_cvt_f32_u32_e32 v6, v4
+	v_add3_u32 v5, v49, v52, 2
+	v_rcp_iflag_f32_e32 v3, v3
+	v_cvt_f32_u32_e32 v14, v5
+	v_add_u32_e32 v7, 1, v49
+	v_lshlrev_b32_e32 v11, 1, v2
+	v_mul_f32_e32 v3, v3, v6
+	v_fmamk_f32 v3, v3, 0x47800000, v66
+	v_cvt_u32_f32_e32 v3, v3
+	v_cvt_f32_u32_e32 v6, v7
+	v_rcp_iflag_f32_e32 v14, v14
+	v_lshl_add_u32 v2, v4, 17, v2
+	v_mul_u32_u24_e32 v4, v3, v11
+	v_sub_u32_e32 v2, v2, v4
+	v_mul_f32_e32 v4, v14, v6
+	v_fmamk_f32 v4, v4, 0x47800000, v66
+	v_cvt_u32_f32_e32 v4, v4
+	v_cmp_ge_u32_e32 vcc, v2, v11
+	v_add_u32_e32 v38, 1, v45
+	v_cvt_f32_u32_e32 v39, v38
+	v_addc_co_u32_e32 v2, vcc, 0, v3, vcc
+	v_lshlrev_b32_e32 v3, 1, v5
+	v_lshl_add_u32 v5, v7, 17, v5
+	v_add3_u32 v7, v51, v54, 2
+	v_cvt_f32_u32_e32 v11, v7
+	v_mul_u32_u24_e32 v6, v4, v3
+	v_sub_u32_e32 v5, v5, v6
+	v_add_u32_e32 v6, 1, v51
+	v_cvt_f32_u32_e32 v14, v6
+	v_rcp_iflag_f32_e32 v11, v11
+	v_cmp_ge_u32_e32 vcc, v5, v3
+	v_add3_u32 v5, v45, v48, 2
+	v_lshl_add_u32 v6, v6, 17, v7
+	v_addc_co_u32_e32 v3, vcc, 0, v4, vcc
+	v_mul_f32_e32 v4, v11, v14
+	v_cvt_f32_u32_e32 v11, v5
+	v_fmamk_f32 v4, v4, 0x47800000, v66
+	v_cvt_u32_f32_e32 v4, v4
+	v_lshlrev_b32_e32 v14, 1, v7
+	v_rcp_iflag_f32_e32 v11, v11
+	v_add_u32_e32 v40, 1, v41
+	v_mul_u32_u24_e32 v7, v4, v14
+	v_sub_u32_e32 v6, v6, v7
+	v_mul_f32_e32 v7, v11, v39
+	v_fmamk_f32 v7, v7, 0x47800000, v66
+	v_cvt_u32_f32_e32 v7, v7
+	v_cmp_ge_u32_e32 vcc, v6, v14
+	v_add3_u32 v14, v43, v46, 2
+	v_lshlrev_b32_e32 v6, 1, v5
+	v_lshl_add_u32 v5, v38, 17, v5
+	v_cvt_f32_u32_e32 v38, v14
+	v_mul_u32_u24_e32 v11, v7, v6
+	v_sub_u32_e32 v5, v5, v11
+	v_add_u32_e32 v11, 1, v43
+	v_cvt_f32_u32_e32 v39, v11
+	v_rcp_iflag_f32_e32 v38, v38
+	v_addc_co_u32_e32 v4, vcc, 0, v4, vcc
+	v_cmp_ge_u32_e32 vcc, v5, v6
+	v_mul_f32_e32 v6, v38, v39
+	v_fmamk_f32 v6, v6, 0x47800000, v66
+	v_addc_co_u32_e32 v5, vcc, 0, v7, vcc
+	v_add3_u32 v7, v41, v44, 2
+	v_cvt_f32_u32_e32 v38, v7
+	v_cvt_u32_f32_e32 v6, v6
+	v_cvt_f32_u32_e32 v41, v40
+	v_lshlrev_b32_e32 v39, 1, v14
+	v_rcp_iflag_f32_e32 v38, v38
+	v_lshl_add_u32 v11, v11, 17, v14
+	v_mul_u32_u24_e32 v14, v6, v39
+	v_sub_u32_e32 v11, v11, v14
+	v_mul_f32_e32 v14, v38, v41
+	v_fmamk_f32 v14, v14, 0x47800000, v66
+	v_cvt_u32_f32_e32 v14, v14
+	v_add3_u32 v37, v19, v37, 2
+	v_cmp_ge_u32_e32 vcc, v11, v39
+	v_cvt_f32_u32_e32 v39, v37
+	v_lshlrev_b32_e32 v11, 1, v7
+	v_lshl_add_u32 v7, v40, 17, v7
+	v_mul_u32_u24_e32 v38, v14, v11
+	v_addc_co_u32_e32 v6, vcc, 0, v6, vcc
+	v_sub_u32_e32 v7, v7, v38
+	v_add_u32_e32 v19, 1, v19
+	v_cvt_f32_u32_e32 v38, v19
+	v_rcp_iflag_f32_e32 v39, v39
+	v_cmp_ge_u32_e32 vcc, v7, v11
+	v_add3_u32 v9, v8, v9, 2
+	v_lshl_add_u32 v19, v19, 17, v37
+	v_addc_co_u32_e32 v7, vcc, 0, v14, vcc
+	v_cvt_f32_u32_e32 v14, v9
+	v_mul_f32_e32 v11, v39, v38
+	v_add_u32_e32 v39, 1, v8
+	v_cvt_f32_u32_e32 v8, v39
+	v_rcp_iflag_f32_e32 v14, v14
+	v_fmamk_f32 v11, v11, 0x47800000, v66
+	v_cvt_u32_f32_e32 v11, v11
+	v_lshlrev_b32_e32 v38, 1, v37
+	v_mul_f32_e32 v8, v14, v8
+	v_fmamk_f32 v8, v8, 0x47800000, v66
+	v_mul_u32_u24_e32 v37, v11, v38
+	v_cvt_u32_f32_e32 v14, v8
+	v_sub_u32_e32 v19, v19, v37
+	v_cmp_ge_u32_e32 vcc, v19, v38
+	s_or_b32 s24, s80, 1
+	v_and_b32_e32 v50, 0xff, v71
+	v_addc_co_u32_e32 v8, vcc, 0, v11, vcc
+	v_lshlrev_b32_e32 v11, 1, v9
+	v_lshl_add_u32 v9, v39, 17, v9
+	v_mul_u32_u24_e32 v19, v14, v11
+	v_sub_u32_e32 v9, v9, v19
+	v_cmp_ge_u32_e32 vcc, v9, v11
+	v_lshrrev_b32_e32 v11, 24, v71
+	v_lshl_or_b32 v82, v11, 8, v50
+	v_addc_co_u32_e32 v9, vcc, 0, v14, vcc
+	v_and_b32_e32 v14, s24, v10
+	v_and_b32_e32 v11, s81, v1
+	v_ffbh_u32_e32 v14, v14
+	v_add_u32_e64 v14, v14, 32 clamp
+	v_ffbh_u32_e32 v11, v11
+	v_and_b32_e32 v39, s81, v13
+	v_min3_u32 v11, v14, v11, 64
+	v_and_b32_e32 v38, s80, v12
+	v_ffbl_b32_e32 v14, v39
+	v_add_u32_e32 v14, 32, v14
+	v_ffbl_b32_e32 v19, v38
+	v_min_u32_e32 v14, v19, v14
+	v_lshlrev_b64 v[40:41], v14, -1
+	v_sub_u32_e32 v11, 63, v11
+	v_not_b32_e32 v14, v41
+	v_cmp_ne_u64_e32 vcc, 0, v[38:39]
+	v_not_b32_e32 v19, v40
+	v_lshlrev_b64 v[38:39], v11, -1
+	v_cndmask_b32_e32 v14, -1, v14, vcc
+	v_cndmask_b32_e32 v19, -1, v19, vcc
+	v_and_b32_e32 v11, v14, v39
+	v_and_b32_e32 v14, v19, v38
+	v_and_b32_e32 v43, s77, v11
+	v_and_b32_e32 v11, 0x80, v71
+	v_and_b32_e32 v42, s76, v14
+	v_cmp_eq_u32_e32 vcc, 0, v11
+	v_and_b32_e32 v14, 64, v71
+	s_mov_b32 s25, s81
+	v_cndmask_b32_e64 v11, v67, 1, vcc
+	v_cmp_eq_u32_e32 vcc, 0, v14
+	v_and_b32_e32 v14, 32, v71
+	s_and_b64 s[8:9], s[24:25], s[76:77]
+	v_cndmask_b32_e64 v19, v67, 1, vcc
+	v_cmp_eq_u32_e32 vcc, 0, v14
+	v_and_b32_e32 v14, 16, v71
+	s_bcnt1_i32_b64 s58, s[8:9]
+	v_cndmask_b32_e64 v44, v67, 1, vcc
+	v_cmp_eq_u32_e32 vcc, 0, v14
+	v_and_b32_e32 v14, 8, v71
+	v_mov_b64_e32 v[40:41], s[58:59]
+	v_cndmask_b32_e64 v45, v67, 1, vcc
+	v_cmp_eq_u32_e32 vcc, 0, v14
+	v_and_b32_e32 v14, 4, v71
+	s_mov_b64 s[8:9], s[74:75]
+	v_cndmask_b32_e64 v46, v67, 1, vcc
+	v_cmp_eq_u32_e32 vcc, 0, v14
+	v_and_b32_e32 v14, 2, v71
+	s_nop 0
+	v_cndmask_b32_e64 v48, v67, 1, vcc
+	v_cmp_eq_u32_e32 vcc, 0, v14
+	v_and_b32_e32 v14, 1, v71
+	s_nop 0
+	v_cndmask_b32_e64 v49, v67, 1, vcc
+	v_cmp_eq_u32_e32 vcc, 0, v14
+	s_nop 1
+	v_cndmask_b32_e64 v47, v67, 1, vcc
+.LBB161_66:
+	v_and_b32_e32 v14, 0xfff, v18
+	v_cndmask_b32_e64 v14, v14, v18, s[2:3]
+	v_lshlrev_b32_e32 v5, 16, v5
+	v_lshl_add_u64 v[38:39], v[14:15], 4, s[70:71]
+	s_and_b64 vcc, s[6:7], s[64:65]
+	v_lshlrev_b32_e32 v14, 16, v3
+	v_or_b32_e32 v3, v5, v4
+	v_lshlrev_b32_e32 v4, 16, v9
+	v_lshlrev_b32_e32 v7, 16, v7
+	v_lshrrev_b32_e32 v54, 24, v71
+	v_bfe_u32 v77, v82, 7, 8
+	v_bfe_u32 v76, v82, 6, 8
+	v_bfe_u32 v75, v82, 5, 8
+	v_bfe_u32 v74, v82, 4, 8
+	v_bfe_u32 v73, v82, 3, 8
+	v_bfe_u32 v72, v82, 2, 8
+	v_bfe_u32 v51, v82, 1, 8
+	v_cndmask_b32_e32 v39, v17, v39, vcc
+	v_cndmask_b32_e32 v38, v16, v38, vcc
+	v_or_b32_e32 v2, v14, v2
+	v_or_b32_e32 v5, v4, v8
+	v_or_b32_e32 v4, v7, v6
+	s_mov_b64 s[78:79], -1
+	s_mov_b32 s92, s91
+	v_mov_b32_e32 v18, v36
+	global_store_dwordx4 v[38:39], v[2:5], off
diff --git a/weath3rb0i_amd/csrc/w3_predict.h b/weath3rb0i_amd/csrc/w3_predict.h
--- a/weath3rb0i_amd/csrc/w3_predict.h
+++ b/weath3rb0i_amd/csrc/w3_predict.h
@@ -105,9 +105,10 @@
     return __builtin_amdgcn_mbcnt_hi((uint32_t)(m >> 32), __builtin_amdgcn_mbcnt_lo((uint32_t)m, 0u));
 }
 
-template <bool GROUPED>
+struct NothingUnder { __device__ __forceinline__ void operator()() const {} };
+template <bool GROUPED, class UNDER = NothingUnder>
 __device__ __forceinline__ void rank_round(uint32_t c0, const uint32_t key[8], const uint64_t M[8], uint64_t seg, bool valid, bool rd,
-                                           uint32_t *tbl, uint32_t p[8], uint32_t fin[8], uint32_t &wmask) {
+                                           uint32_t *tbl, uint32_t p[8], uint32_t fin[8], uint32_t &wmask, UNDER under = UNDER()) {
     __asm__ volatile("" ::: "memory");
     const uint64_t gt = lane_gt_mask();
     const int lane = threadIdx.x & 63;
@@ -115,6 +116,7 @@
     uint32_t basev[8];
 #pragma unroll
     for (int j = 0; j < 8; j++) basev[j] = tbl[j * 256 + key[j]];
+    under();
 #pragma unroll
     for (int j = 0; j < 8; j++) {
         const uint64_t Mj = M[j] & seg;
@@ -713,6 +715,44 @@
     }
 }
 
+struct RankFront {
+    uint32_t i, c0, g;
+    uint32_t key[8], inc[8];
+    uint64_t vm, heads, seg;
+    uint32_t g_first, g_last;
+    uint32_t nseg;
+};
+template <int NBYTES>
+__device__ __forceinline__ RankFront rank_front(uint2 rec, uint32_t base, uint32_t len, uint32_t prev_g) {
+    const uint32_t lane = threadIdx.x & 63;
+    RankFront f;
+    const bool valid = lane < (base < len ? len - base : 0u);
+    const uint32_t w = valid ? rec.y : 0u;
+    f.i = rec.x;
+    f.c0 = w & 0xFFu;
+    f.g = NBYTES == 1 ? ((w >> 8) & 0xFFu) : ((w >> 8) & 0xFFFFu);
+    const uint32_t ck = NBYTES == 1 ? ((w >> 16) & 0xFFu) : (w >> 24);
+    const uint32_t w16 = (ck << 8) | f.c0;
+    const uint32_t gprev = (uint32_t)__builtin_amdgcn_update_dpp((int)prev_g, (int)f.g, 0x138, 0xF, 0xF, false);
+    f.vm = __ballot(valid);
+    f.heads = __ballot(valid && f.g != gprev) | 1ull;
+    const uint64_t hle = f.heads & (lane_lt_mask() | (1ull << lane));
+    const int start = 63 - __clzll((long long)hle);
+    const uint64_t hgt = f.heads & lane_gt_mask();
+    const uint64_t below_end = hgt ? ((1ull << (__ffsll((long long)hgt) - 1)) - 1ull) : ~0ull;
+    f.seg = below_end & ~((1ull << start) - 1ull) & f.vm;
+#pragma unroll
+    for (int j = 0; j < 8; j++) {
+        f.key[j] = (w16 >> (8 - j)) & 0xFFu;
+        f.inc[j] = ((f.c0 >> (7 - j)) & 1u) ? 0x10000u : 1u;
+    }
+    const int lastlane = f.vm ? 63 - __clzll((long long)f.vm) : 0;
+    f.g_last = readlane_u32(f.g, lastlane);
+    f.g_first = readlane_u32(f.g, 0);
+    f.nseg = (uint32_t)__popcll(f.heads & f.vm);
+    return f;
+}
+
 template <int NBYTES, int NW = 1, int PF = W3_PF, bool FAULT = false>
 __global__ void __launch_bounds__(64 * NW) k_rank_sorted(PredictArgs a) {
     __shared__ uint32_t tbl_[NW][8 * 256];
@@ -743,8 +783,12 @@
         uint32_t open_g = 0xFFFFFFFFu;
         const uint32_t last = len - 1u;
         uint2 rn[PF];
-#pragma unroll
-        for (int r = 0; r < PF; r++) rn[r] = perm[min((uint32_t)(r * 64 + lane), last)];
+        const uint2 r_0 = perm[min((uint32_t)lane, last)];
+        uint2 r_next = perm[min((uint32_t)(64 + lane), last)];
+#pragma unroll
+        for (int r = 0; r < PF; r++) rn[r] = perm[min((uint32_t)((2 + r) * 64 + lane), last)];
+        RankFront f = rank_front<NBYTES>(r_0, 0u, len, open_g);
+        __builtin_amdgcn_s_waitcnt(0x0070);
         for (uint32_t bbase = 0; bbase < len; bbase += 64u * (uint32_t)PF) {
             __asm__ volatile("" ::: "memory");
             __builtin_amdgcn_wave_barrier();
@@ -753,41 +797,28 @@
             __asm__ volatile("" ::: "memory");
             __builtin_amdgcn_wave_barrier();
 #pragma unroll
-            for (int r = 0; r < PF; r++) rn[r] = perm[min(bbase + (uint32_t)((PF + r) * 64 + lane), last)];
+            for (int r = 0; r < PF; r++) rn[r] = perm[min(bbase + (uint32_t)((PF + 2 + r) * 64 + lane), last)];
 #pragma unroll 1
           for (uint32_t rr = 0; rr < (uint32_t)PF; rr++) {
             const uint32_t base = bbase + rr * 64u;
             if (base >= len) break;
-            const uint32_t e = base + lane;
-            const bool valid = e < len;
-            const uint2 r_c = st_r[rr * 64u + lane];
-            const uint32_t i = r_c.x; const uint32_t w = valid ? r_c.y : 0u;
-            const uint32_t c0 = w & 0xFFu;
-            const uint32_t g = NBYTES == 1 ? ((w >> 8) & 0xFFu) : ((w >> 8) & 0xFFFFu);
-            const uint32_t ck = NBYTES == 1 ? ((w >> 16) & 0xFFu) : (w >> 24);
-            const uint32_t w16 = (ck << 8) | c0;
-            uint32_t gprev = __shfl_up(g, 1, 64);
-            if (lane == 0) gprev = open_g;
-            const uint64_t vm = __ballot(valid);
-            const uint64_t heads = __ballot(valid && g != gprev) | 1ull;
-            const uint64_t hle = heads & (lane_lt_mask() | (1ull << lane));
-            const int start = 63 - __clzll((long long)hle);
-            const uint64_t hgt = heads & lane_gt_mask();
-            const uint64_t below_end = hgt ? ((1ull << (__ffsll((long long)hgt) - 1)) - 1ull) : ~0ull;
-            const uint64_t seg = below_end & ~((1ull << start) - 1ull) & vm;
-            uint32_t key[8], p[8];
-#pragma unroll
-            for (int j = 0; j < 8; j++) key[j] = (w16 >> (8 - j)) & 0xFFu;
+            const RankFront c = f;
+            const bool valid = base + lane < len;
+            const uint2 r_n = r_next;
+            const auto front_ahead = [&]() {
+                r_next = st_r[rr * 64u + lane];
+                f = rank_front<NBYTES>(r_n, base + 64u, len, c.g_last);
+                __builtin_amdgcn_sched_barrier(0);
+            };
+            uint32_t p[8];
             uint32_t *vt = tbl;
-            const int lastlane = 63 - __clzll((long long)vm);
-            const uint32_t g_last = readlane_u32(g, lastlane);
-            uint64_t hm = heads & vm;
-            if (!exact && (uint32_t)__popcll(hm) <= a.maxseg) {
+            uint64_t hm = c.heads & c.vm;
+            if (!exact && c.nseg <= a.maxseg) {
                 uint32_t v[8];
 #pragma unroll
                 for (int j = 0; j < 8; j++) v[j] = 0u;
                 __asm__ volatile("" ::: "memory");
-                if (dirty && readlane_u32(g, 0) != open_g) {
+                if (dirty && c.g_first != open_g) {
 #pragma unroll
                     for (int k = 0; k < 32; k++) vt[k * 64 + lane] = 0u;
                     dirty = false;
@@ -799,7 +830,11 @@
                     const int en = hm ? __ffsll((long long)hm) - 1 : 64;
                     const bool in = valid && lane >= st && lane < en;
                     __asm__ volatile("" ::: "memory");
-                    if (in) atomic_round(vt, c0, key, true, v);
+                    if (in) {
+#pragma unroll
+                        for (int j = 0; j < 8; j++)
+                            v[j] = __hip_atomic_fetch_add(&vt[j * 256 + c.key[j]], c.inc[j], __ATOMIC_RELAXED, __HIP_MEMORY_SCOPE_WORKGROUP);
+                    }
                     __asm__ volatile("" ::: "memory");
                     if (hm) {
                         if (carried) {
@@ -807,12 +842,13 @@
                             for (int k = 0; k < 32; k++) vt[k * 64 + lane] = 0u;
                         } else if (in) {
 #pragma unroll
-                            for (int j = 0; j < 8; j++) vt[j * 256 + key[j]] = 0u;
+                            for (int j = 0; j < 8; j++) vt[j * 256 + c.key[j]] = 0u;
                         }
                     }
                     carried = false;
                 }
                 __asm__ volatile("" ::: "memory");
+                front_ahead();
                 if constexpr (FAULT) {
                     if (64u - (lo + base) < 64u && (a.fault_block == 0xFFFFFFFFu || a.fault_block == b)) v[0] = (uint32_t)__shfl_xor((int)v[0], 1, 64);
                 }
@@ -822,26 +858,26 @@
             } else {
                 uint32_t fin[8], wm;
                 uint64_t M[8];
-                match_windows<8>(w16, M);
-                rank_round<true>(c0, key, M, seg, valid, g == open_g, vt, p, fin, wm);
-                if (g_last != open_g && dirty) {
+                match_windows<8>((c.key[0] << 8) | c.c0, M);
+                rank_round<true>(c.c0, c.key, M, c.seg, valid, c.g == open_g, vt, p, fin, wm, front_ahead);
+                if (c.g_last != open_g && dirty) {
 #pragma unroll
                     for (int k = 0; k < 32; k++) vt[k * 64 + lane] = 0u;
                     dirty = false;
                 }
                 __builtin_amdgcn_wave_barrier();
-                if (valid && g == g_last) {
+                if (valid && c.g == c.g_last) {
 #pragma unroll
                     for (int j = 0; j < 8; j++)
-                        if ((wm >> j) & 1u) vt[j * 256 + key[j]] = fin[j];
+                        if ((wm >> j) & 1u) vt[j * 256 + c.key[j]] = fin[j];
                 }
                 __asm__ volatile("" ::: "memory");
                 __builtin_amdgcn_wave_barrier();
             }
             dirty = true;
-            open_g = g_last;
+            open_g = c.g_last;
             {
-                uint4 *dst = (valid && !(a.dbg_flags & 1u)) ? a.P + (off + ((a.dbg_flags & 4u) ? (i & 0xFFFu) : i)) : a.sink + lane;
+                uint4 *dst = (valid && !(a.dbg_flags & 1u)) ? a.P + (off + ((a.dbg_flags & 4u) ? (c.i & 0xFFFu) : c.i)) : a.sink + lane;
                 *dst = pack_p(p);
             }
           }
```

After: 14300 (median of 2 runs). Within noise of the previous version (+0.1%).
